# waveygang/wfmash

Measured on AMD Instinct MI355X. Metric: aligned bases/sec (whole node) + CIGAR-identical rate vs CPU ref, higher is better.
Workload: dtype int32; 1 GPU; C3: 64 synthetic 5%-divergence 50kb segment pairs per GPU, WFA-only (BiWFA gap-affine-2p 5,8,2,24,1; mappings pre-supplied); pairs_per_gpu=64, pairs_total=64, parallelism=records sharded over 1 GPU(s)

## Files before the change

### include/wfmash_hip.h

```cpp
#ifndef WFMASH_HIP_H_
#define WFMASH_HIP_H_

#include <stddef.h>
#include <stdint.h>

#ifdef __cplusplus
extern "C" {
#endif

#define WFM_OK              0
#define WFM_E_NODEVICE     (-1)
#define WFM_E_HIP          (-2)
#define WFM_E_ARG          (-3)
#define WFM_E_NOMEM        (-4)
#define WFM_E_UNSUPPORTED  (-5)
#define WFM_E_ARENA        (-6)

#define WFM_ST_OK            0
#define WFM_ST_UNREACHABLE (-300)
#define WFM_ST_OOM         (-200)
#define WFM_ST_MAX_SCORE   (-100)

#define WFMASH_HIP_VERSION "wfmash-hip-0.3"

// ... 164 lines not shown
#define WFM_COV_TILE 4096
#define WFM_COV_SCAN_BLOCK 1024
int  wfm_coverage_create(wfm_handle_t* h, uint64_t n_bases, wfm_coverage_t** cov);
void wfm_coverage_free(wfm_coverage_t* cov);
int  wfm_coverage_add(wfm_handle_t* h, wfm_coverage_t* cov, const wfm_cov_prob_t* probs, size_t n, const uint32_t* runs, size_t n_runs_total,
                      uint32_t* flags_out);
int  wfm_coverage_export(wfm_handle_t* h, wfm_coverage_t* cov, wfm_cov_entry_t** entries, size_t* n);
int  wfm_coverage_import(wfm_handle_t* h, wfm_coverage_t* cov, const wfm_cov_entry_t* entries, size_t n);
int  wfm_coverage_intervals(wfm_handle_t* h, wfm_coverage_t* cov, wfm_cov_interval_t** iv, size_t* n, uint64_t totals[3]);
void wfm_coverage_free_list(void* p);

typedef struct wfm_liftset wfm_liftset_t;
typedef struct { uint64_t start, end; } wfm_lift_iv_t;
typedef struct { uint32_t problem, interval, p0, p1, t0, t1, eq, x; } wfm_lift_t;
typedef struct { uint32_t flags, n_runs; uint64_t first, count; } wfm_liftcall_t;
#define WFM_LIFT_SPANS 2u
#define WFM_LIFT_SCAN_BLOCK 1024
int  wfm_liftset_create(wfm_handle_t* h, const wfm_lift_iv_t* iv, size_t n, uint64_t n_bases, wfm_liftset_t** out);
void wfm_liftset_free(wfm_liftset_t* s);
int  wfm_lift_runs(wfm_handle_t* h, const wfm_liftset_t* s, const wfm_cov_prob_t* probs, size_t n, const uint32_t* runs, size_t n_runs_total,
                   wfm_lift_t** lifts, size_t* n_lifts, wfm_liftcall_t* per);
void wfm_free_lifts(wfm_lift_t* p);

typedef struct wfm_pav wfm_pav_t;
typedef struct { uint64_t base, runs_off; uint32_t n_runs, group; } wfm_pav_prob_t;
typedef struct { uint64_t start; uint32_t length, group; } wfm_pav_seg_t;
#define WFM_PAV_SPANS 2u
#define WFM_PAV_SCAN_BLOCK 1024
int  wfm_pav_create(wfm_handle_t* h, uint64_t n_bases, uint32_t n_groups, wfm_pav_t** pav);
void wfm_pav_free(wfm_pav_t* pav);
int  wfm_pav_add(wfm_handle_t* h, wfm_pav_t* pav, const wfm_pav_prob_t* probs, size_t n, const uint32_t* runs, size_t n_runs_total,
                 uint32_t* flags_out);
int  wfm_pav_union(wfm_handle_t* h, wfm_pav_t* pav);
int  wfm_pav_export(wfm_handle_t* h, wfm_pav_t* pav, wfm_pav_seg_t** segs, size_t* n);
int  wfm_pav_import(wfm_handle_t* h, wfm_pav_t* pav, const wfm_pav_seg_t* segs, size_t n);
int  wfm_pav_matrix(wfm_handle_t* h, wfm_pav_t* pav, const wfm_lift_iv_t* iv, size_t n_iv, uint32_t* out);
int  wfm_pav_counts(const wfm_pav_t* pav, uint64_t out[3]);
void wfm_pav_free_list(void* p);

#define WFM_OPT_NOT_CHECKED 1u
#define WFM_OPT_SKIPPED     2u
#define WFM_OPT_CHEAPER     4u
#define WFM_OPT_UNREACHED   8u
typedef struct {
  uint32_t flags; int32_t dp_score;
  int32_t  band_lo, band_hi;
  uint64_t cells;
} wfm_optcheck_t;
#define WFM_OPT_BAND_C1   256
#define WFM_OPT_BAND_C4   1024
#define WFM_OPT_REG_MAX   4096
#define WFM_OPT_ROWS_MB   256
int wfm_check_optimal(wfm_handle_t* h, const wfm_penalties_t* pen, const wfm_seqset_t* s,
                      const wfm_result_t* res, uint64_t max_cells , wfm_optcheck_t* out);

void wfm_set_concurrent_calls(wfm_handle_t* h, int other_calls);

#define WFM_PF_ROOT_AGAIN   1u
#define WFM_PF_JOB_AGAIN    2u
#define WFM_PF_BASE_RETRY   4u
#define WFM_PF_BASE_RETRY2  8u
#define WFM_PF_BYTE_KERNEL 16u
#define WFM_PF_P2_ROUNDS   32u
#define WFM_PF_RING_KERNEL 64u
#define WFM_PF_BASE_TILES 128u
#define WFM_PF_RING_GROWN 256u
size_t wfm_get_problem_flags(const wfm_handle_t* h, uint32_t* out, size_t n);

enum {
  WFM_TC_JOBS = 0,
  WFM_TC_EXACT_ENDS = 1,
  WFM_TC_FINE_RERUNS = 2,
  WFM_TC_GAP_RERUNS = 3,
  WFM_TC_RING3 = 4,
  WFM_TC_BLOCKS_COARSE = 5,
  WFM_TC_BLOCKS_FINE = 6,
  WFM_TC_LEFT_BAND = 7,
  WFM_TC_REUSE_RESUMED = 8,
  WFM_TC_REUSE_FALLBACKS = 9,
  WFM_TC_REUSE_KEEPS = 10,
  WFM_TC_REUSE_TOUCHED = 11,
  WFM_TC_REUSE_FELL_OTHER = 12,
  WFM_TC_PLANNED_ENDS = 13,
  WFM_TILE_COUNTERS = 14
};
size_t wfm_get_tile_counters(const wfm_handle_t* h, uint64_t* out, size_t n);

size_t wfm_trim_device_cache(void);

int  wfm_get_stats(const wfm_handle_t* h, wfm_stats_t* out);
size_t wfm_get_busy_intervals(const wfm_handle_t* h, double* start_end_ms, size_t cap);


int  wfm_hash_kmers(wfm_handle_t* h, const char* seq, int64_t len, int k,
                    uint64_t* hash, int8_t* strand);

typedef struct {
  uint64_t hash;
  int64_t  wpos;
  int64_t  wpos_end;
  int32_t  seqId;
  int16_t  strand;
  int16_t  pad_;
} wfm_minmer_t;

int  wfm_sketch_fragments(wfm_handle_t* h, const char* seq, int64_t seq_len,
                          const int64_t* frag_off, const int32_t* frag_len, size_t n,
                          int k, int s, int32_t seq_id,
                          wfm_minmer_t* out, int32_t* out_count);

typedef struct {
  int64_t  pos;
  uint64_t hash;
  int32_t  seqId;
  int8_t   side;
  int8_t   pad_[3];
} wfm_interval_point_t;

typedef struct wfm_index wfm_index_t;
typedef struct {
  int64_t  n_windows;
  int64_t  n_kept;
  int64_t  n_unique;
  int64_t  n_points;
  uint64_t threshold;
  int64_t  filtered;
  int32_t  adjusted;
  int32_t  pad_;
} wfm_index_info_t;
int  wfm_index_build(wfm_handle_t* h, const wfm_minmer_t* minmers, int64_t n, double max_kmer_freq, wfm_index_t** out);
void wfm_index_free(wfm_handle_t* h, wfm_index_t* ix);
int  wfm_index_info(const wfm_index_t* ix, wfm_index_info_t* out);
int  wfm_index_download(wfm_handle_t* h, const wfm_index_t* ix, uint64_t* uhash, int64_t* poff,
                        wfm_interval_point_t* points, wfm_minmer_t* minmers);

int  wfm_index_replicate(wfm_handle_t* src, const wfm_index_t* ix, wfm_handle_t* dst, wfm_index_t** out);

int  wfm_index_upload(wfm_handle_t* h, const uint64_t* uhash, const int64_t* poff, int64_t n_unique,
                      const wfm_interval_point_t* points, const wfm_minmer_t* minmers, int64_t n_kept,
                      wfm_index_t** out);

int64_t wfm_add_minmers(wfm_handle_t* h, const char* seq, int64_t len, int k, int w, int s, int32_t seq_id,
                        wfm_minmer_t* out, int64_t cap);

int64_t wfm_add_minmers_multi(wfm_handle_t* h, const char* const* seqs, const int64_t* lens, const int32_t* seq_ids,
                              int64_t nseq, int k, int w, int s, int threads, wfm_minmer_t* out, int64_t cap, int64_t* counts);

int wfm_index_build_sequences(wfm_handle_t* h, const char* const* seqs, const int64_t* lens, const int32_t* seq_ids,
                              int64_t nseq, int k, int w, int s, int threads, double max_kmer_freq,
                              wfm_index_t** out, int64_t* n_windows);

typedef struct wfm_minmer_part wfm_minmer_part_t;
int  wfm_sketch_part(wfm_handle_t* h, const char* const* seqs, const int64_t* lens, const int32_t* seq_ids, int64_t nseq,
                     int k, int w, int s, int threads, wfm_minmer_part_t** out);
int64_t wfm_minmer_part_info(const wfm_minmer_part_t* part, int64_t* n_records, int64_t* counts, int64_t cap);
int64_t wfm_minmer_part_download(wfm_handle_t* h, const wfm_minmer_part_t* part, wfm_minmer_t* out, int64_t cap);
void wfm_minmer_part_free(wfm_minmer_part_t* part);

typedef struct { int32_t part; int32_t seq; } wfm_part_seq_t;
#define WFM_GATHER_TILE 2048
int  wfm_index_build_parts(wfm_handle_t* h, const wfm_minmer_part_t* const* parts, int nparts, const wfm_part_seq_t* order,
                           int64_t norder, double max_kmer_freq, wfm_index_t** out, int64_t* n_windows);

int64_t wfm_prefilter_kmers(wfm_handle_t* h, const char* seq, int64_t len, int k, int w, int s, double c_factor,
                            uint32_t* pos, uint64_t* hash, int8_t* strand, int64_t cap);

int64_t wfm_finish_records(wfm_handle_t* h, const wfm_minmer_t* raw, int64_t n, int w, wfm_minmer_t* out, int64_t cap,
// ... 90 lines not shown
```

### wfmash_amd/capi.py

```python
import ctypes as C
import os

import numpy as np

_HERE = os.path.dirname(os.path.abspath(__file__))
LIB_PATH = os.environ.get("WFM_LIB_PATH") or os.path.join(_HERE, "libwfmash_hip.so")

WFM_MODE_END2END_BIWFA = 0
WFM_MODE_ENDSFREE = 1
WFM_MODE_END2END_UNI = 2
WFM_MODE_MASK = 0xff
WFM_MODE_SCORE_ONLY = 0x100
WFM_MODE_SCORE_LIMIT = 0x200
WFM_ST_MAX_SCORE = -100

DEFAULT_PEN = (5, 8, 2, 24, 1)
WFM_PF_ROOT_AGAIN, WFM_PF_JOB_AGAIN, WFM_PF_BASE_RETRY, WFM_PF_BASE_RETRY2, WFM_PF_BYTE_KERNEL, WFM_PF_P2_ROUNDS, WFM_PF_RING_KERNEL, WFM_PF_BASE_TILES = 1, 2, 4, 8, 16, 32, 64, 128
WFM_PF_RING_GROWN = 256
TILE_COUNTERS = ("jobs", "exact_ends", "fine_reruns", "gap_reruns", "ring3", "blocks_coarse", "blocks_fine", "left_band",
                 "reuse_resumed", "reuse_fallbacks", "reuse_keeps", "reuse_touched", "reuse_fell_other", "planned_ends")

EXPORTS = [
    "wfm_create", "wfm_destroy", "wfm_last_error", "wfm_device_name",
    "wfm_align_arena_bytes", "wfm_align_batch", "wfm_upload_sequences",
    "wfm_free_sequences", "wfm_align_resident", "wfm_get_stats",
    "wfm_hash_kmers", "wfm_sketch_fragments", "wfm_add_minmers",
    "wfm_index_build", "wfm_index_free", "wfm_index_info", "wfm_index_download",
    "wfm_map_l1", "wfm_map_l2", "wfm_map_fragments", "wfm_minhash_sketch", "wfm_add_minmers_multi",
    "wfm_prefilter_kmers", "wfm_index_build_sequences", "wfm_index_upload",
    "wfm_index_replicate", "wfm_device_count", "wfm_finish_records",
    "wfm_align_batch_rle", "wfm_align_resident_rle", "wfm_free_runs", "wfm_score_bounds", "wfm_get_busy_intervals", "wfm_trim_device_cache", "wfm_map_fragments_ordered", "wfm_map_sequence_cache", "wfm_selftest_dpp", "wfm_selftest_arena_growth", "wfm_set_concurrent_calls", "wfm_get_problem_flags",
    "wfm_get_tile_counters",
    "wfm_streaming_minmers", "wfm_index_build_streaming",
    "wfm_sketch_part", "wfm_minmer_part_info", "wfm_minmer_part_download", "wfm_minmer_part_free", "wfm_index_build_parts",
    "wfm_seqstore_create", "wfm_seqstore_free", "wfm_seqstore_add", "wfm_seqstore_info",
    "wfm_upload_sequence_refs", "wfm_align_refs_rle", "wfm_download_sequences",
    "wfm_check_runs", "wfm_check_optimal", "wfm_left_align_runs", "wfm_cs_strings", "wfm_free_cs",
    "wfm_call_variants", "wfm_free_variants",
    "wfm_coverage_create", "wfm_coverage_free", "wfm_coverage_add", "wfm_coverage_export", "wfm_coverage_import", "wfm_coverage_intervals",
    "wfm_coverage_free_list",
    "wfm_liftset_create", "wfm_liftset_free", "wfm_lift_runs", "wfm_free_lifts",
    "wfm_pav_create", "wfm_pav_free", "wfm_pav_add", "wfm_pav_union", "wfm_pav_export", "wfm_pav_import", "wfm_pav_matrix", "wfm_pav_counts",
    "wfm_pav_free_list",
    "wfm_sketch_intersections",
]
ISECT_LDS_MAX = 4096
WFM_CK_NOT_CHECKED, WFM_CK_BAD_RUN, WFM_CK_SPANS, WFM_CK_M_DIFFERS, WFM_CK_X_EQUAL, WFM_CK_SCORE, WFM_CK_COUNTS = 1, 2, 4, 8, 16, 32, 64
CK_NAMES = ("NOT_CHECKED", "BAD_RUN", "SPANS", "M_DIFFERS", "X_EQUAL", "SCORE", "COUNTS")
CHECK_SLICE = 16384
WFM_LA_NOT_DONE, WFM_LA_SPANS = 1, 2
WFM_CS_SHORT, WFM_CS_LONG = 0, 1
WFM_CS_NOT_DONE, WFM_CS_SPANS = 1, 2
WFM_CS_SLICE = 16384
WFM_VAR_SNV, WFM_VAR_INS, WFM_VAR_DEL = 0, 1, 2
WFM_VAR_MASKED = 256
WFM_VAR_NOT_DONE, WFM_VAR_SPANS = 1, 2
WFM_VAR_SLICE = 16384
WFM_COV_SPANS = 2
WFM_COV_TILE = 4096
WFM_COV_SCAN_BLOCK = 1024
WFM_LIFT_SPANS = 2
WFM_LIFT_SCAN_BLOCK = 1024
WFM_PAV_SPANS = 2
WFM_PAV_SCAN_BLOCK = 1024
WFM_OPT_NOT_CHECKED, WFM_OPT_SKIPPED, WFM_OPT_CHEAPER, WFM_OPT_UNREACHED = 1, 2, 4, 8
OPT_NAMES = ("NOT_CHECKED", "SKIPPED", "CHEAPER", "UNREACHED")
OPT_BAND_C1, OPT_BAND_C4, OPT_REG_MAX = 256, 1024, 4096
OPT_ROWS_MB = 256
SEQ_GATHER_CHUNK = 16384


class Penalties(C.Structure):
    _fields_ = [("x", C.c_int32), ("o1", C.c_int32), ("e1", C.c_int32),
                ("o2", C.c_int32), ("e2", C.c_int32)]


class Problem(C.Structure):
    _fields_ = [("pattern", C.c_char_p), ("plen", C.c_int32),
                ("text", C.c_char_p), ("tlen", C.c_int32),
                ("mode", C.c_int32),
                ("pattern_begin_free", C.c_int32), ("pattern_end_free", C.c_int32),
                ("text_begin_free", C.c_int32), ("text_end_free", C.c_int32),
                ("score_hint", C.c_int32), ("pad_", C.c_int32)]


class ProblemRef(C.Structure):
    _fields_ = [("pattern", C.c_char_p), ("text", C.c_char_p),
                ("pattern_off", C.c_int64), ("text_off", C.c_int64),
                ("pattern_seq", C.c_int32), ("text_seq", C.c_int32),
                ("plen", C.c_int32), ("tlen", C.c_int32),
                ("mode", C.c_int32),
                ("pattern_revcomp", C.c_int32), ("text_revcomp", C.c_int32),
                ("pattern_begin_free", C.c_int32), ("pattern_end_free", C.c_int32),
                ("text_begin_free", C.c_int32), ("text_end_free", C.c_int32),
                ("score_hint", C.c_int32)]


class Result(C.Structure):
    _fields_ = [("status", C.c_int32), ("score", C.c_int32),
                ("ops_off", C.c_uint64), ("ops_len", C.c_uint32),
                ("n_runs", C.c_uint32), ("cells", C.c_uint64)]


# ... 2053 lines not shown
```

### wfmash_amd/csrc/wfa_device.h

```cpp
#ifndef WFM_WFA_DEVICE_H_
#define WFM_WFA_DEVICE_H_

#include <hip/hip_runtime.h>
#include <stdint.h>

#include "wfa_rows.h"

namespace wfm {

constexpr int WF_NULL = -(1 << 30);
constexpr int RING = 32;
constexpr int RMASK = RING - 1;
constexpr int RING_BIG = 128;

enum { C_M = 0, C_I1 = 1, C_I2 = 2, C_D1 = 3, C_D2 = 4 };
enum { OP_M = 0, OP_X = 1, OP_I = 2, OP_D = 3 };
enum { BT_I1_EXT = 8, BT_I2_EXT = 16, BT_D1_EXT = 32, BT_D2_EXT = 64 };

constexpr int WFM_DEV_UNREACHABLE = -300;
constexpr int WFM_DEV_OVERFLOW = -2;
constexpr int WFM_DEV_BAND = -4;
constexpr int WFM_DEV_P2_NOTHING = -6;
constexpr int WFM_DEV_LIMIT = -7;
constexpr int WFM_DEV_P2_MORE = -5;

struct DevPen { int x, o1, e1, o2, e2; };

struct BpJob {
  int64_t p_fwd, t_fwd, p_rev, t_rev;
  int64_t ring_off;
  int32_t pl, tl;
  int32_t comp_begin, comp_end;
  int32_t width;
  int32_t koff;
  int32_t resume_s;
  int32_t fmax0, rmax0;
  int32_t band;
  int32_t resume_sr;
  int32_t last_fwd;
  int32_t sub;
  int32_t best0;
  int32_t packed;
  int32_t limit;
};
static_assert(sizeof(BpJob) == 104, "BpJob::limit fills the struct's tail padding: the job arrays keep their stride");

struct TileJob {
  int64_t p_fwd, t_fwd, p_rev, t_rev;
  int64_t ring_in, ring_out;
  int32_t pl, tl;
  int32_t comp_begin, comp_end;
  int32_t width, koff;
  int32_t s0;
  int32_t active;
  int32_t fmax, rmax;
  int32_t nblocks;
  int32_t mode;
  int32_t tf, tr;
  int32_t last_fwd;
  int32_t packed;
  int64_t p2_off;
  int32_t w2, koff2;
  int32_t sub;
  int32_t fine_s;
  int64_t ring_prev;
  int32_t prev_ok;
  int32_t reran;
  int32_t plan_sum;
  int32_t plan_deep;
};
static_assert(sizeof(TileJob) == 160, "TileJob::plan_sum and its padding behind reran: no field the tile kernels read has moved");
__host__ __device__ inline bool tile_plan_enter(TileJob& J, int T) {
  if (J.plan_sum <= 0) return false;
  const int sf = (J.plan_sum + 1) / 2, sr = J.plan_sum / 2;
  if ((sf - 1) / T * T != J.s0) return false;
  J.tf = sf - J.s0; J.tr = sr - J.s0; J.last_fwd = J.plan_sum & 1;
  J.mode = (J.ring_prev >= 0 && J.prev_ok && !J.plan_deep && (J.tf < J.tr ? J.tf : J.tr) < 26) ? 6 : 1;
  return true;
}
__host__ __device__ inline bool tile_plan_short_next(const TileJob& J, int T) {
  if (J.plan_sum <= 0 || !J.plan_deep || J.mode != 0) return false;
  const int sf = (J.plan_sum + 1) / 2, sr = J.plan_sum / 2, b0 = (sf - 1) / T * T;
  return b0 == J.s0 + T && sr - b0 < 26;
}

struct KeepTask {
  int32_t* dst;
  int32_t job, dir;
  int32_t expect_s;
  int32_t kmin, n;
  int32_t pad_;
};
struct RestoreTask {
  const int32_t* src;
  int32_t job, dir;
  int32_t s_k, kmin, n;
  int32_t slack;
};
void launch_keep(const int32_t* ring, const TileJob* jobs, const KeepTask* tasks, int ntasks, int max_n, hipStream_t st);
void launch_restore(int32_t* ring, const TileJob* jobs, const RestoreTask* tasks, int32_t* out, int ntasks, int max_n, hipStream_t st);

constexpr int P2K = 32;
constexpr int P2ROWS = SNAP_ROWS + P2K;
constexpr int P2TESTS = 2 * P2K;
constexpr int P2ENT = RING * 5;
struct P2Job {
  int64_t ring_in;
  int64_t p2_off;
  int32_t width, koff;
  int32_t w2, koff2;
  int32_t pl, tl;
  int32_t sf, sr, last_fwd;
  int32_t sub, best0;
  int32_t nblk;
  int64_t bm_off;
};

struct BpResult {
  int32_t status;
  int32_t score, score_fwd, score_rev, k_fwd, off_fwd, comp;
  int32_t steps;
  uint64_t cells;
  int32_t steps_p1;
  uint32_t ticks_p1, ticks_p2;
  int32_t pad_;
  uint32_t ticks_list, ticks_pick;
  uint32_t work_items, pad2_;
};

struct BaseJob {
  int64_t p_off, t_off;
  int64_t pre_off;
  int64_t bt_off;
  int64_t ring_off;
  int64_t rle_end;
  int32_t pl, tl;
  int32_t comp_begin, comp_end;
  int32_t endsfree, pbf, pef, tbf, tef;
  int32_t smax, kmin, width;
  int32_t type;
  int32_t pad_;
  int32_t score_only;
};
static_assert(sizeof(BaseJob) == 112, "BaseJob::score_only fills the struct's tail padding: the job arrays keep their stride");

struct BaseResult {
  int32_t status;
  int32_t score;
  int32_t nruns;
  int32_t pad_;
  uint64_t cells;
};

struct Base2TJob {
  BaseJob b;
  int64_t snap_in, snap_out;
  int32_t ntiles, core;
  int32_t task0;
  int32_t s0;
  int32_t done;
  int32_t end_s, end_k, end_off;
};
struct Base2TTask { int32_t job, tile; };
constexpr int B2T_ROWS = 32;
constexpr int B2T_THREADS = 512;
void launch_base2t_block(const uint32_t* pk, int32_t* a32, uint8_t* a8, const Base2TJob* jobs, const Base2TTask* tasks, unsigned long long* tile_key,
                         int32_t* tile_off, int ntasks, int T, hipStream_t st);
void launch_base2t_advance(Base2TJob* jobs, const unsigned long long* tile_key, const int32_t* tile_off, int njobs, int T, int32_t* active_slot, hipStream_t st);
void launch_base2t_finish(const int32_t* a32, const uint8_t* a8, uint32_t* rle, const Base2TJob* jobs, BaseResult* res, int njobs, hipStream_t st);

struct BoundJob { int64_t p_off, t_off; int32_t pl, tl; };
void launch_bound(const uint8_t* seq, const BoundJob* jobs, int32_t* out, int njobs, DevPen pen, hipStream_t st);

struct SeqRev { int64_t p_fwd, p_rev, t_fwd, t_rev; int32_t plen, tlen; };
void launch_reverse(uint8_t* seq, const SeqRev* jobs, int njobs, int pad, hipStream_t st);
struct SeqGatherTask { const uint8_t* src; uint8_t* dst; int32_t len, pad; int32_t reverse, complement; };
void launch_seq_gather(const SeqGatherTask* tasks, int64_t ntasks, hipStream_t st);
struct CheckProb {
  int64_t p_off, t_off;
  uint64_t run_off;
  uint32_t n_runs;
  int32_t plen, tlen;
  int32_t pbf, pef, tbf, tef;
  int32_t res_score;
  uint32_t res_ops_len;
  int32_t skip;
};
struct CheckTask { int32_t prob, slice; };
void launch_check(const uint8_t* seq, const uint32_t* runs, const CheckProb* probs, int nprob, const CheckTask* tasks, int64_t ntasks,
                  uint32_t* ops_pre, uint32_t* p_pre, uint32_t* t_pre, uint32_t* cmp_ops, unsigned long long* keys, void* out, DevPen pen,
                  hipStream_t st);
struct LaProb {
  int64_t p_off, t_off;
  uint64_t run_off, out_off, gap_off;
  uint32_t n_runs, n_gaps;
  int32_t plen, tlen;
  int32_t skip, pad_;
};
struct LaGap { int64_t s_off; uint32_t g, len, prob, run; };
// ... 18 lines not shown
                      hipStream_t st);
struct CovProb {
  uint64_t base, runs_off;
  uint32_t n_runs, pad_;
};
void launch_cov_add(const uint32_t* runs, const CovProb* probs, int nprob, int32_t* d, unsigned long long n_bases, uint32_t* flags, hipStream_t st);
void launch_cov_tile_offsets(const int32_t* d, unsigned long long ntiles, uint32_t* tile_cnt, unsigned long long* sums, unsigned long long* tile_off,
                             hipStream_t st);
void launch_cov_write(const int32_t* d, const unsigned long long* tile_off, unsigned long long tile_a, unsigned long long tile_b,
                      unsigned long long out_base, void* out, hipStream_t st);
void launch_cov_import(const void* ent, unsigned long long n, int32_t* d, hipStream_t st);
void launch_cov_intervals(const void* ent, unsigned long long m, unsigned long long* sums, unsigned long long* carry, unsigned long long prev_pos,
                          unsigned long long n_bases, int last, void* iv, unsigned long long* totals, hipStream_t st);
struct LiftProb {
  uint64_t base, runs_off, pre_off;
  uint32_t n_runs, pad_;
};
struct LiftWin {
  uint64_t lo, hi, count;
  uint32_t flags, plen;
};
void launch_lift_pm(const void* iv, unsigned long long n, unsigned long long* maxs, unsigned long long* pm, hipStream_t st);
void launch_lift_index(const uint32_t* runs, const LiftProb* probs, int nprob, const void* iv, const unsigned long long* pm, unsigned long long n_iv,
                       unsigned long long n_bases, void* pre, LiftWin* win, unsigned long long* off, hipStream_t st);
void launch_lift_write(const uint32_t* runs, const LiftProb* probs, const void* iv, const void* pre, const LiftWin* win, const unsigned long long* off,
                       uint32_t ka, uint32_t kb, void* out, hipStream_t st);
struct PavProb {
  uint64_t base, runs_off;
  uint32_t n_runs, group;
};
void launch_pav_count(const uint32_t* runs, const PavProb* probs, int nprob, unsigned long long n_bases, uint32_t n_groups, uint32_t* flags,
                      unsigned long long* cnt, unsigned long long* off, hipStream_t st);
void launch_pav_write(const uint32_t* runs, const PavProb* probs, int nprob, const uint32_t* flags, const unsigned long long* off,
                      unsigned long long* ks, unsigned long long* ke, hipStream_t st);
hipError_t pav_sort(void* tmp, size_t* tmp_bytes, const unsigned long long* ks, unsigned long long* ks2, const unsigned long long* ke,
                    unsigned long long* ke2, unsigned long long n, unsigned end_bit, hipStream_t st);
void launch_pav_runmax(unsigned long long* ke, unsigned long long n, unsigned long long* aux, hipStream_t st);
void launch_pav_compact(const unsigned long long* ks, const unsigned long long* rm, unsigned long long n, unsigned long long* aux,
                        unsigned long long* uks, unsigned long long* uke, hipStream_t st);
void launch_pav_prefix(const unsigned long long* uks, const unsigned long long* uke, unsigned long long m, unsigned long long* aux,
                       unsigned long long* C, hipStream_t st);
void launch_pav_matrix(const unsigned long long* uks, const unsigned long long* uke, const unsigned long long* C, unsigned long long m, const void* iv,
                       unsigned long long ra, unsigned long long rb, uint32_t n_groups, uint32_t* out, hipStream_t st);
struct OptProb {
  int64_t p_off, t_off, row_off;
  int32_t plen, tlen;
  int32_t pbf, pef, tbf, tef;
  int32_t band_lo, band_hi;
};
void launch_optcheck(const uint8_t* seq, const OptProb* probs, int nprob, int form, int32_t* rows, int32_t* out, DevPen pen, hipStream_t st);
void launch_seq_normalize(uint8_t* seq, int64_t nbytes, hipStream_t st);
void launch_seq_pack(const uint8_t* seq, uint32_t* pk, int64_t nwords, int64_t nbytes, const SeqRev* jobs, int njobs, int32_t* flag, hipStream_t st);
constexpr int64_t PK_PAD_WORDS = 2048 + 64;
void launch_tile2(const uint32_t* pk, int32_t* ring, const TileJob* jobs, const TileTask* tasks, int32_t* mak, int ntasks, int threads, int T, int variants, hipStream_t st);
#ifndef WFM_TILE_SLOTS_WIDE
#define WFM_TILE_SLOTS_WIDE 16
#endif
constexpr int TILE_SLOTS_WAVE1 = 2, TILE_SLOTS_SMALL = 4, TILE_SLOTS_WIDE = WFM_TILE_SLOTS_WIDE;
constexpr int tile_fine_slots(int threads) { return threads <= 64 ? TILE_SLOTS_WAVE1 : (threads <= 128 ? TILE_SLOTS_SMALL : TILE_SLOTS_WIDE); }
bool tile2_coarse_maxima();
void launch_tile2_p2(const uint32_t* pk, int32_t* ring, const TileJob* jobs, const TileTask* tasks, int ntasks, int threads, int32_t* p2, hipStream_t st);
int selftest_dpp(int* host_out128, hipStream_t st);
void launch_base2(const uint32_t* pk, int32_t* a32, uint8_t* a8, uint32_t* rle, const BaseJob* jobs, BaseResult* res, int njobs, int threads, hipStream_t st);
void launch_bp(const uint8_t* seq, int32_t* ring, const BpJob* jobs, BpResult* res, int njobs, int threads,
               DevPen pen, int scope, int ring_rows, hipStream_t st);
void launch_tile_init(const uint8_t* seq, int32_t* ring, const TileJob* jobs, int32_t* mak0, int njobs, int ring_rows, hipStream_t st);
void launch_tile(const uint8_t* seq, int32_t* ring, const TileJob* jobs, const TileTask* tasks, int32_t* mak, int ntasks,
                 int threads, int T, int Wt, size_t lds_bytes, DevPen pen, int scope, int ring_rows, hipStream_t st);
void launch_tile_advance(TileJob* jobs, int32_t* mak, int njobs, int T, DevPen pen, int exact, int coarse, int launched, hipStream_t st);
void launch_tile_reg(const uint8_t* seq, int32_t* ring, const TileJob* jobs, const TileTask* tasks, int32_t* mak, int ntasks,
                     int threads, int T, int C, bool cut, hipStream_t st);
void launch_tile_p2(const uint8_t* seq, int32_t* ring, const TileJob* jobs, const TileTask* tasks, int ntasks, int threads,
                    int32_t* p2, bool cut, hipStream_t st);
void launch_p2_to_ring(int32_t* ring, const int32_t* p2, const P2Job* jobs, int njobs, hipStream_t st);
struct RingWidenJob {
  const int32_t* src;
  int32_t* dst;
  int32_t src_w, src_koff;
  int32_t dst_w, dst_koff;
  int32_t klo, khi;
};
void launch_ring_widen(const RingWidenJob* jobs, int njobs, int max_dst_w, int ring_rows, hipStream_t st);
void launch_p2_blockmax(const int32_t* ring, const int32_t* p2, const P2Job* jobs, int32_t* bmax, int32_t* p2max, int njobs, hipStream_t st);
void launch_p2_overlap(const int32_t* ring, const int32_t* p2, const P2Job* jobs, const int32_t* p2max, const int32_t* bmax, int32_t* pbmax,
                       BpResult* res, int njobs, int threads, int max_nblk, DevPen pen, int scope, hipStream_t st);
void launch_base(const uint8_t* seq, int32_t* a32, uint8_t* a8, uint32_t* rle, const BaseJob* jobs, BaseResult* res,
                 int njobs, DevPen pen, bool wide, int ring_rows, hipStream_t st);
void launch_compact(const uint32_t* rle, const int64_t* off, const int64_t* cap, uint32_t* out, unsigned long long* total,
                    int64_t* out_start, int32_t* out_count, int nprob, hipStream_t st);

}
#endif
```

### wfmash_amd/csrc/wfa_host.hip

```cpp
#include <hip/hip_runtime.h>

#include <algorithm>
#include <chrono>
#include <climits>
#include <cstdio>
#include <cstring>
#include <atomic>
#include <mutex>
#include <string>
#include <thread>
#include <vector>

#include "../../include/wfmash_hip.h"
#include "wfa_host_shared.h"
#include "wfa_plan.h"
#include "wfa_optband.h"

#ifdef WFM_PROFILE_SECTIONS
namespace wfm { void read_sections(long long* out); }
#endif
namespace wfm { void p2_counters(unsigned long long* out); }
namespace {

using namespace wfm;
// ... 774 lines not shown
  wfm_handle* h = p.h;
  uint64_t unique_level = 0;
  for (size_t i = 0; i < p.n; ++i) {
    const TileJob& t = p.tj[i];
    const int sf_end = t.mode == 2 ? t.s0 + t.tf : t.s0, sr_end = t.mode == 2 ? t.s0 + t.tr : t.s0;
    if (p.ru && p.ru->bad[i]) continue;
    unique_level += (uint64_t)cells_sum(t.pl, t.tl, t.sub, p.s_begin[i] + 1, sf_end) + (uint64_t)cells_sum(t.pl, t.tl, t.sub, p.s_begin[i] + 1, sr_end);
  }
  h->stats.cells_tile_unique += unique_level;
  for (size_t i = 0; i < p.n; ++i) {
    const TileJob& t = p.tj[i];
    BpJob& j = p.jobs[(size_t)p.tiled[i]];
    j.ring_off = t.ring_in;
    p.ring2[i] = t.ring_out;
    j.resume_s = t.s0;
    j.resume_sr = -1; j.last_fwd = 0;
    h->tile_ctr[WFM_TC_EXACT_ENDS] += t.mode == 2;
    h->tile_ctr[WFM_TC_PLANNED_ENDS] += t.mode == 2 && t.plan_sum > 0;
    h->tile_ctr[WFM_TC_LEFT_BAND] += t.mode == 3 && !(p.ru && p.ru->bad[i]);
    if (t.mode == 3) {
      j.resume_s = -3; j.resume_sr = t.s0; j.fmax0 = p.fmax[i]; j.rmax0 = p.rmax[i];
      continue;
    }
    if (t.mode == 2) {
      j.resume_s = t.s0 + t.tf;
      j.resume_sr = t.s0 + t.tr;
      j.last_fwd = t.last_fwd;
    }
    j.fmax0 = p.fmax[i]; j.rmax0 = p.rmax[i];
  }
  if (p.cfg.debug) fprintf(stderr, "[wfm] level %u: tiled %zu jobs, %u blocks of %d scores (Wt %d), %.3f ms; %.3e cells computed on %.3e lane-steps (%.0f %% of the lanes hold a cell), %.3e of them in the result (the block in which a job's wavefronts meet runs twice); launches of the packed kernel without / with per-score maxima %u / %u, mode-5 reruns %u, mode-6 reruns %u\n", level, p.n, p.blocks, p.T, p.cfg.Wt, p.tile_ms,
                           (double)p.tile_cells - cells_before, p.lane_cells, p.lane_cells > 0 ? 100.0 * ((double)p.tile_cells - cells_before) / p.lane_cells : 0.0, (double)unique_level,
                           p.launches_coarse, p.launches_fine, p.reruns5, p.reruns6);
}

int run_tiled_phase(wfm_handle* h, wfm_seqset* S, const DevPen& dp, int scope, const TileCfg& cfg, int T, bool refine,
                    std::vector<BpJob>& jobs, const std::vector<int>& tiled, std::vector<int64_t>& ring2,
                    double& tile_ms, uint64_t& tile_cells, uint32_t level, const std::vector<int32_t>* fine_from = nullptr,
                    const std::vector<int64_t>* ring3 = nullptr, ReuseCtl* reuse = nullptr, const std::vector<int32_t>* plan_from = nullptr) {
  const size_t n = tiled.size();
  if (n == 0) return WFM_OK;
  const double cells_before = (double)tile_cells;
  TilePhase p{h, S, dp, scope, cfg, T, refine, jobs, tiled, ring2, tile_ms, tile_cells, n};
  p.ru = refine ? nullptr : reuse;
  int rc = init_tile_jobs(p, fine_from, ring3, plan_from);
  if (rc != WFM_OK) return rc;
  if (p.n_active) {
    HIPCHK(h, hipMemcpyAsync(h->tilejobs.p, p.tj.data(), n * sizeof(TileJob), hipMemcpyHostToDevice, h->stream));
    HIPCHK(h, hipMemsetAsync(h->tilemak.p, 0, n * 2 * (size_t)T * sizeof(int32_t), h->stream));
    p.chunk = std::max(1, std::min(cfg.chunk, (int)h->tile_ev.size() / 2));
    p.got.resize(n); p.pjobs.resize(n);
    p.rules = TilePlanRules{cfg.threads, cfg.C, T, p.chunk, cfg.Wt - 2 * T, cfg.reg, cfg.fine, cfg.reg && cfg.exact && tile2_coarse_maxima(), p.any_planned};
    auto clk = [] { return std::chrono::steady_clock::now(); };
    auto msd = [](std::chrono::steady_clock::time_point a, std::chrono::steady_clock::time_point b) { return std::chrono::duration<double, std::milli>(b - a).count(); };
    double ms_prep = 0, ms_launch = 0, ms_wait = 0, ms_post = 0;
    while (p.n_active) {
      const auto tq0 = clk();
      if ((rc = drop_leavers(p)) != WFM_OK) return rc;
      if (!p.n_active) break;
      if ((rc = plan_tile_tasks(p)) != WFM_OK) return rc;
      const auto tq1 = clk();
      if ((rc = launch_chunk(p)) != WFM_OK) return rc;
      const auto tq2 = clk();
      HIPCHK(h, hipStreamSynchronize(h->stream));
      const auto tq3 = clk();
      if ((rc = time_chunk(p)) != WFM_OK) return rc;
      account_chunk(p);
      settle_keeps(p);
      if ((rc = restore_kept(p)) != WFM_OK) return rc;
      ms_prep += msd(tq0, tq1); ms_launch += msd(tq1, tq2); ms_wait += msd(tq2, tq3); ms_post += msd(tq3, clk());
    }
    if (cfg.debug > 1)
      fprintf(stderr, "[wfm] level %u tile phase, host side: task lists %.2f ms, launches %.2f ms, waiting for the device %.2f ms, bookkeeping %.2f ms\n", level, ms_prep, ms_launch, ms_wait, ms_post);
  }
  hand_back(p, level, cells_before);
  return WFM_OK;
}


struct P2Chunk {
  wfm_handle* h; wfm_seqset* S; const DevPen& dp; int scope; const TileCfg& cfg; std::vector<BpJob>& jobs;
  const std::vector<int>& cand; const std::vector<int64_t>& ring_other; std::vector<BpResult>& res; double& ms_out;
  std::vector<BpResult>& carry; std::vector<char>& has_carry; bool may_continue; std::vector<int>& again;
  std::vector<P2PlanJob> pcand;
  P2ChunkPlan plan;
  size_t i0 = 0, n = 0;
  std::vector<TileJob> tj;
  std::vector<P2Job> pj;
  std::vector<BpResult> got;
  float ms = 0;
};

void fill_p2_chunk(P2Chunk& c, size_t i0) {
  const size_t budget = std::max<size_t>(c.h->mem_budget / 4, (size_t)64 << 20);
  plan_p2_chunk(c.pcand.data(), c.pcand.size(), i0, P2K, P2ROWS, budget, c.cfg.threads, c.cfg.Wt - 2 * P2K, c.plan);
  c.i0 = i0; c.n = c.plan.geo.size();
  c.tj.clear(); c.pj.clear();
  for (size_t q = 0; q < c.n; ++q) {
    const BpJob& j = c.jobs[(size_t)c.cand[i0 + q]];
    const P2Geometry& g = c.plan.geo[q];
    TileJob t = tile_job_from(j);
    t.ring_out = c.ring_other[i0 + q];
    t.mode = 4; t.tf = j.resume_s; t.tr = j.resume_sr; t.last_fwd = j.last_fwd;
    t.p2_off = (int64_t)g.p2_off; t.w2 = (int32_t)g.w2; t.koff2 = g.koff2;
    P2Job pq{};
    pq.ring_in = j.ring_off; pq.p2_off = (int64_t)g.p2_off; pq.width = j.width; pq.koff = j.koff; pq.w2 = (int32_t)g.w2; pq.koff2 = g.koff2;
    pq.pl = j.pl; pq.tl = j.tl; pq.sf = j.resume_s; pq.sr = j.resume_sr; pq.last_fwd = j.last_fwd; pq.sub = j.sub; pq.best0 = j.best0;
    pq.nblk = (int32_t)g.nblk; pq.bm_off = (int64_t)g.bm_off;
    c.tj.push_back(t); c.pj.push_back(pq);
  }
}

int launch_p2_chunk(P2Chunk& c) {
  wfm_handle* h = c.h;
  wfm_seqset* S = c.S;
  const size_t n = c.n, elems = c.plan.elems, bm_elems = c.plan.bm_elems, n_pk = c.plan.tiles.n_pk;
  const std::vector<TileTask>& tasks = c.plan.tiles.tasks;
  const int threads_c = c.plan.threads_c;
  if (h->p2rows.ensure(elems + 16) || h->p2max.ensure(n * 2 * P2ROWS * 5) || h->p2bmax.ensure(bm_elems + 16) || h->p2pbmax.ensure(bm_elems + 16) ||
      h->p2jobs.ensure(n) || h->tilejobs.ensure(n) || h->tiletasks.ensure(tasks.size()) || h->bpres.ensure(std::max(n, c.jobs.size()))) {
    h->err = "out of device memory (phase-2 rows)"; return WFM_E_NOMEM;
  }
  HIPCHK(h, hipMemcpyAsync(h->tilejobs.p, c.tj.data(), n * sizeof(TileJob), hipMemcpyHostToDevice, h->stream));
  HIPCHK(h, hipMemcpyAsync(h->p2jobs.p, c.pj.data(), n * sizeof(P2Job), hipMemcpyHostToDevice, h->stream));
  HIPCHK(h, hipMemcpyAsync(h->tiletasks.p, tasks.data(), tasks.size() * sizeof(TileTask), hipMemcpyHostToDevice, h->stream));
  HIPCHK(h, hipEventRecord(h->ev0, h->stream));
  bool any_cut = false;
  for (const TileJob& t : c.tj) any_cut |= t.sub != SUB_NONE;
  if (n_pk) launch_tile2_p2(S->d_pk, h->ring.p, h->tilejobs.p, h->tiletasks.p, (int)n_pk, threads_c, h->p2rows.p, h->stream);
  if (tasks.size() > n_pk) launch_tile_p2(S->d_seq, h->ring.p, h->tilejobs.p, h->tiletasks.p + n_pk, (int)(tasks.size() - n_pk), threads_c, h->p2rows.p, any_cut, h->stream);
  launch_p2_blockmax(h->ring.p, h->p2rows.p, h->p2jobs.p, h->p2bmax.p, h->p2max.p, (int)n, h->stream);
  static const int p2_threads = getenv("WFM_P2_THREADS") ? atoi(getenv("WFM_P2_THREADS")) : 0;
  launch_p2_overlap(h->ring.p, h->p2rows.p, h->p2jobs.p, h->p2max.p, h->p2bmax.p, h->p2pbmax.p, h->bpres.p, (int)n,
                    p2_threads > 0 ? p2_threads : 1024, (int)(c.plan.maxw2 >> 6) + 1, c.dp, c.scope, h->stream);
  HIPCHK(h, hipGetLastError());
  HIPCHK(h, hipEventRecord(h->ev1, h->stream));
  c.got.resize(n);
  HIPCHK(h, hipMemcpyAsync(c.got.data(), h->bpres.p, n * sizeof(BpResult), hipMemcpyDeviceToHost, h->stream));
  HIPCHK(h, hipStreamSynchronize(h->stream));
  HIPCHK(h, hipEventElapsedTime(&c.ms, h->ev0, h->ev1));
  c.ms_out += c.ms;
  if (h->call_base) {
    float t0 = 0;
    HIPCHK(h, hipEventElapsedTime(&t0, h->call_base, h->ev0));
    h->bp_iv.emplace_back(t0, t0 + c.ms);
  }
  return WFM_OK;
}

int dump_p2_job(P2Chunk& c) {
  wfm_handle* h = c.h;
  const std::vector<BpResult>& got = c.got;
  const size_t q = std::min<size_t>((size_t)c.cfg.p2_dump, c.n - 1);
  std::vector<int32_t> rm((size_t)2 * P2ROWS * 5);
  HIPCHK(h, hipMemcpy(rm.data(), h->p2max.p + q * 2 * P2ROWS * 5, rm.size() * 4, hipMemcpyDeviceToHost));
  const P2Job& pjq = c.pj[q];
  fprintf(stderr, "[wfm] p2 dump job %zu: pl %d tl %d sf %d sr %d last_fwd %d sub %d w2 %d nblk %d -> status %d score %d (fwd %d rev %d comp %d k %d) rounds %d\n", q, pjq.pl, pjq.tl, pjq.sf,
          pjq.sr, pjq.last_fwd, pjq.sub, pjq.w2, pjq.nblk, got[q].status, got[q].score, got[q].score_fwd, got[q].score_rev, got[q].comp, got[q].k_fwd, got[q].pad_);
  for (int d = 0; d < 2; ++d)
    for (int r = 0; r < P2ROWS; r += 3) {
      const int32_t* m = rm.data() + ((size_t)d * P2ROWS + r) * 5;
      fprintf(stderr, "[wfm]   dir %d row %d (s = %d): max M %d I1 %d I2 %d D1 %d D2 %d\n", d, r, (d == 0 ? pjq.sf : pjq.sr) - RNG_BACK + r, m[0], m[1], m[2], m[3], m[4]);
    }
  return WFM_OK;
}

void print_p2_chunk(const P2Chunk& c) {
  const std::vector<BpResult>& got = c.got;
  const std::vector<P2Job>& pj = c.pj;
  const size_t n = c.n;
  int more = 0;
  double tk = 0, tc = 0, rd = 0; uint32_t tkmax = 0; int rdmax = 0;
  for (const BpResult& r : got) { more += r.status == WFM_DEV_P2_MORE; tk += r.ticks_p2; tc += r.ticks_p1; rd += r.pad_; tkmax = std::max(tkmax, r.ticks_p2); rdmax = std::max(rdmax, r.pad_); }
  fprintf(stderr, "[wfm] phase 2 from rows computed ahead: %zu jobs, widest %zu columns, %zu tiles of %d threads, %.3f ms, %d left to the step kernel; walk per job: %.1f rounds (max %d), %.0f us (max %.0f), of which cells stage %.0f us\n",
          n, c.plan.maxw2, c.plan.tiles.tasks.size(), c.plan.threads_c, c.ms, more, rd / n, rdmax, tk / n / 100.0, tkmax / 100.0, tc / n / 100.0);
  size_t qs = 0;
  for (size_t q = 0; q < n; ++q) if (got[q].ticks_p2 > got[qs].ticks_p2) qs = q;
  fprintf(stderr, "[wfm]   slowest walk: pl %d tl %d sub %d w2 %d nblk %d: %d rounds, %.0f us = listing %.0f + cells %.0f (incl. listing) + pick %.0f, %u blocks listed, status %d\n", pj[qs].pl, pj[qs].tl,
          pj[qs].sub == SUB_NONE ? -1 : pj[qs].sub, pj[qs].w2, pj[qs].nblk, got[qs].pad_, got[qs].ticks_p2 / 100.0, got[qs].ticks_list / 100.0, got[qs].ticks_p1 / 100.0, got[qs].ticks_pick / 100.0,
          got[qs].work_items, got[qs].status);
}

int continue_p2_chunk(P2Chunk& c) {
  wfm_handle* h = c.h;
  std::vector<BpResult>& got = c.got;
  std::vector<P2Job> mj;
  for (size_t q = 0; q < c.n; ++q) {
    const size_t jq = (size_t)c.cand[c.i0 + q];
    BpJob& j = c.jobs[jq];
    if (got[q].status == WFM_DEV_P2_NOTHING) { got[q] = c.carry[jq]; continue; }
    if (got[q].status != WFM_DEV_P2_MORE) continue;
    if (got[q].comp >= 0) {
      c.carry[jq] = got[q]; c.carry[jq].status = 0; c.has_carry[jq] = 1;
      j.best0 = got[q].score;
    }
    if (!c.may_continue || (j.band > 0 && std::max(j.resume_s, j.resume_sr) + 2 * P2K + 2 > j.band)) continue;
    mj.push_back(c.pj[q]);
    j.resume_s += P2K; j.resume_sr += P2K;
    c.again.push_back((int)(c.i0 + q));
  }
  if (!mj.empty()) {
    HIPCHK(h, hipMemcpyAsync(h->p2jobs.p, mj.data(), mj.size() * sizeof(P2Job), hipMemcpyHostToDevice, h->stream));
    launch_p2_to_ring(h->ring.p, h->p2rows.p, h->p2jobs.p, (int)mj.size(), h->stream);
    HIPCHK(h, hipGetLastError());
    HIPCHK(h, hipStreamSynchronize(h->stream));
  }
  for (size_t q = 0; q < c.n; ++q) c.res[(size_t)c.cand[c.i0 + q]] = got[q];
  return WFM_OK;
}

int run_p2_phase(wfm_handle* h, wfm_seqset* S, const DevPen& dp, int scope, const TileCfg& cfg, std::vector<BpJob>& jobs,
                 const std::vector<int>& cand, const std::vector<int64_t>& ring_other, std::vector<BpResult>& res, double& ms_out,
                 std::vector<BpResult>& carry, std::vector<char>& has_carry, bool may_continue, std::vector<int>& again) {
  if (cand.empty()) return WFM_OK;
  P2Chunk c{h, S, dp, scope, cfg, jobs, cand, ring_other, res, ms_out, carry, has_carry, may_continue, again};
  for (int q : cand) {
    const BpJob& j = jobs[(size_t)q];
    c.pcand.push_back(P2PlanJob{j.pl, j.tl, j.sub, j.resume_s, j.resume_sr, j.packed});
  }
  for (size_t i0 = 0; i0 < cand.size(); i0 += c.n) {
    fill_p2_chunk(c, i0);
    int rc = launch_p2_chunk(c);
    if (rc != WFM_OK) return rc;
    if (cfg.p2_dump_on && (rc = dump_p2_job(c)) != WFM_OK) return rc;
    h->stats.p2_launches++;
    h->stats.p2_jobs += (uint32_t)c.n;
    if (cfg.debug) print_p2_chunk(c);
    if ((rc = continue_p2_chunk(c)) != WFM_OK) return rc;
  }
  return WFM_OK;
}


struct Knobs {
  static int num(const char* name, int dflt) { const char* e = getenv(name); return e ? atoi(e) : dflt; }
  bool use_hints = num("WFM_SCORE_HINT", 1) != 0;
  bool use_bound = use_hints && num("WFM_BOUND", 1) != 0;
  int slack_env = num("WFM_SUB_SLACK", -1);
  bool ring3_on = num("WFM_TILE_RING3", 1) != 0, p2_on = num("WFM_P2", 1) != 0;
  int p2_rounds = std::max(1, num("WFM_P2_ROUNDS", 64));
  int fine_margin = num("WFM_TILE_FINE_MARGIN", 48);
  int coarse_min_blocks = num("WFM_TILE_COARSE_MIN_BLOCKS", 32), coarse_max_jobs = num("WFM_TILE_COARSE_MAX_JOBS", 128);
  bool planned_end = num("WFM_TILE_PLANNED_END", 1) != 0 && slack_env < (1 << 28);
  bool tile_v2 = num("WFM_TILE_V2", 1) != 0;
  bool band_on = num("WFM_BAND", 1) != 0;
  int band_root = std::max(64, num("WFM_BAND_ROOT", 4096));
  int resume_margin = num("WFM_RESUME_MARGIN", SNAP_ROWS);
  bool reuse = num("WFM_REUSE", 1) != 0 && slack_env < (1 << 28);
  int reuse_min_blocks = std::max(1, num("WFM_REUSE_MIN_BLOCKS", 8));
  int reuse_every = std::max(1, num("WFM_REUSE_EVERY", 2)), reuse_slack = std::max(0, num("WFM_REUSE_TOUCH_SLACK", 0));
  int reuse_levels = num("WFM_REUSE_LEVELS", 8);
  int debug = env_debug();
};

struct Chunk {
  std::vector<BpJob> jobs;
  std::vector<int32_t> node_of;
  size_t ring_elems = 0, end = 0;
  int maxw = 0;
  std::vector<int> tiled, tiled_r;
  std::vector<int64_t> ring2, ring3, ring2_r;
  std::vector<int32_t> fine_from, fine_r, snap_r;
  std::vector<int32_t> plan_from;
  std::vector<size_t> ring_third;
  std::vector<char> grown_job, resume_bad, has_carry;
  std::vector<ReuseUse> reuse;
  std::vector<int32_t> keep_upto;
  std::vector<char> reuse_bad;
  std::vector<std::vector<int32_t>> kept[2];
  std::vector<BpResult> res, carry;
  std::vector<int> rest, more_set;
  void clear() {
    jobs.clear(); node_of.clear(); ring_elems = 0; maxw = 0;
    tiled.clear(); ring2.clear(); ring3.clear(); ring_third.clear(); fine_from.clear();
    tiled_r.clear(); ring2_r.clear(); fine_r.clear(); snap_r.clear(); grown_job.clear();
    reuse.clear(); keep_upto.clear(); plan_from.clear();
  }
};

struct AlignCall {
  wfm_handle* h;
  const wfm_penalties_t* pen;
  wfm_seqset* S;
  size_t first, last;
  wfm_result_t* out;
  char* ops_arena;
  size_t arena_bytes, arena_base;
  std::vector<uint32_t>* runs_out;
  uint32_t* pflags;
  int scope;
  DevPen dp;
  const Knobs knobs;
  TileCfg tcfg;
  BaseCfg bcfg;
  int RR;
  RingRules rules;
  std::vector<int32_t> prob_status;
  std::vector<uint64_t> prob_cells;
  std::vector<int32_t> prob_score;
  std::vector<Node> bp_nodes, base_nodes, next_bp;
  uint32_t level = 0;
  Chunk ck;
  LevelTimer tm;
  double wall_tile = 0, wall_base = 0;
  uint64_t band_retries = 0, band_jobs = 0, roots_banded = 0, roots_out = 0, hint_retries = 0, limit_out = 0;
  uint64_t grown_jobs = 0, grown_widened = 0, grown_restarts = 0;
  int64_t grown_maxband = 0;
  size_t ring_peak = 0;
  GrownSnaps snaps;
  KeepStore keeps;
  uint64_t reuse_children = 0, reuse_found = 0, reuse_taken = 0;
  uint64_t keep_bytes = 0, restore_bytes = 0;
  uint64_t reuse_full_rings = 0;
};

void make_roots(AlignCall& c) {
  for (size_t i = c.first; i < c.last; ++i) {
    const ProbMeta& pm = c.S->meta[i];
    Node nd{};
    nd.prob = (int32_t)i; nd.pb = 0; nd.pl = pm.plen; nd.tb = 0; nd.tl = pm.tlen;
    nd.cb = C_M; nd.ce = C_M; nd.score_rem = INT_MAX; nd.endsfree = 0;
    nd.sub = SUB_NONE; nd.hinted = 0;
// ... 175 lines not shown
  k.resume_bad.assign(k.jobs.size(), 0);
  if (k.tiled_r.empty()) return WFM_OK;
  std::vector<RingWidenJob> wj;
  int maxw_dst = 0;
  for (size_t q = 0; q < k.tiled_r.size(); ++q) {
    BpJob& j = k.jobs[(size_t)k.tiled_r[q]];
    const GrownSnap& sn = c.snaps.v[(size_t)k.snap_r[q] - 1];
    wj.push_back(RingWidenJob{sn.d, h->ring.p + j.ring_off, sn.w, sn.koff, j.width, j.koff, -(sn.s0 + 8), sn.s0 + 8});
    maxw_dst = std::max(maxw_dst, j.width);
    j.resume_s = sn.s0; j.resume_sr = -1; j.fmax0 = sn.fmax; j.rmax0 = sn.rmax;
  }
  if (h->widenjobs.ensure(wj.size())) { h->err = "out of device memory (ring arena)"; return WFM_E_NOMEM; }
  HIPCHK(h, hipMemcpyAsync(h->widenjobs.p, wj.data(), wj.size() * sizeof(RingWidenJob), hipMemcpyHostToDevice, h->stream));
  launch_ring_widen(h->widenjobs.p, (int)wj.size(), maxw_dst, c.RR, h->stream);
  HIPCHK(h, hipGetLastError());
  HIPCHK(h, hipStreamSynchronize(h->stream));
  for (int32_t id : k.snap_r) c.snaps.drop(id);
  return WFM_OK;
}

int run_chunk_tiles(AlignCall& c) {
  wfm_handle* h = c.h;
  Chunk& k = c.ck;
  const TileCfg& tcfg = c.tcfg;
  double tms = 0; uint64_t tcells = 0;
  const auto tw0 = std::chrono::steady_clock::now();
  ReuseCtl ru;
  ru.store = &c.keeps; ru.slack = c.knobs.reuse_slack; ru.min_blocks = c.knobs.reuse_min_blocks;
  ru.use = k.reuse; ru.upto = k.keep_upto;
  for (size_t q = 0; q < k.tiled.size(); ++q) {
    const Node& nd = c.bp_nodes[(size_t)k.node_of[(size_t)k.tiled[q]]];
    ru.meet.push_back(nd.score_rem != INT_MAX ? nd.score_rem / 2 : 0);
  }
  {
    std::vector<ReuseKeeper> kp;
    for (size_t q = 0; q < k.tiled.size(); ++q) {
      const BpJob& j = k.jobs[(size_t)k.tiled[q]];
      if (k.keep_upto[q] > 0) kp.push_back(ReuseKeeper{j.pl, j.tl, k.keep_upto[q] == INT_MAX ? (j.pl + j.tl) / 16 : k.keep_upto[q]});
    }
    c.keeps.cap_bytes = h->mem_budget / 8;
    const int chunk_blocks = std::max(1, std::min(tcfg.chunk, (int)h->tile_ev.size() / 2));
    ru.cadence = kp.empty() ? 0 : reuse_fit_cadence(kp.data(), kp.size(), reuse_cadence(c.knobs.reuse_every, chunk_blocks), tcfg.T, c.keeps.cap_bytes);
  }
  const bool any_reuse = ru.cadence > 0 || std::any_of(ru.use.begin(), ru.use.end(), [](const ReuseUse& u) { return u.keep > 0; });
  int rc = run_tiled_phase(h, c.S, c.dp, c.scope, tcfg, tcfg.T, false, k.jobs, k.tiled, k.ring2, tms, tcells, c.level, &k.fine_from, &k.ring3, any_reuse ? &ru : nullptr, &k.plan_from);
  k.reuse_bad.assign(k.jobs.size(), 0);
  k.kept[0].assign(k.jobs.size(), {}); k.kept[1].assign(k.jobs.size(), {});
  if (any_reuse && !ru.bad.empty())
    for (size_t q = 0; q < k.tiled.size(); ++q) {
      k.reuse_bad[(size_t)k.tiled[q]] = ru.bad[q];
      for (int d = 0; d < 2; ++d) k.kept[d][(size_t)k.tiled[q]].swap(ru.kept[d][q]);
    }
  c.keep_bytes += ru.keep_bytes; c.restore_bytes += ru.restore_bytes;
  if (rc == WFM_OK && tcfg.T_refine > 0 && tcfg.T_refine < tcfg.T && !(tcfg.reg && tcfg.exact))
    rc = run_tiled_phase(h, c.S, c.dp, c.scope, tcfg, tcfg.T_refine, true, k.jobs, k.tiled, k.ring2, tms, tcells, c.level);
  if (rc == WFM_OK && !k.tiled_r.empty()) {
    std::vector<int> from_s(k.tiled_r.size());
    for (size_t q = 0; q < k.tiled_r.size(); ++q) from_s[q] = k.jobs[(size_t)k.tiled_r[q]].resume_s;
    rc = run_tiled_phase(h, c.S, c.dp, c.scope, tcfg, tcfg.T, true, k.jobs, k.tiled_r, k.ring2_r, tms, tcells, c.level, &k.fine_r);
    for (size_t q = 0; rc == WFM_OK && q < k.tiled_r.size(); ++q) {
      BpJob& j = k.jobs[(size_t)k.tiled_r[q]];
      const bool exact_end = j.resume_s >= 0 && j.resume_sr >= 0;
      if (tcfg.reg && tcfg.exact && ((exact_end && std::min(j.resume_s, j.resume_sr) - from_s[q] < c.knobs.resume_margin) || (j.resume_s >= 0 && j.resume_sr < 0 && j.resume_s == from_s[q]))) {
        j.resume_s = -3; j.resume_sr = -1;
        k.resume_bad[(size_t)k.tiled_r[q]] = 1;
      }
      k.tiled.push_back(k.tiled_r[q]); k.ring2.push_back(k.ring2_r[q]);
    }
  }
  c.wall_tile += std::chrono::duration<double, std::milli>(std::chrono::steady_clock::now() - tw0).count();
  if (rc != WFM_OK) return rc;
  c.tm.bp_ms += tms; c.tm.tile_ms += tms;
  h->stats.cells_bp += tcells; h->stats.cells_tile += tcells;
  return WFM_OK;
}

int run_chunk_p2(AlignCall& c) {
  wfm_handle* h = c.h;
  Chunk& k = c.ck;
  k.res.assign(k.jobs.size(), BpResult{});
  k.rest.clear(); k.more_set.clear();
  std::vector<int> cand;
  std::vector<int64_t> other;
  std::vector<char> is_cand(k.jobs.size(), 0);
  if (c.knobs.p2_on && c.tcfg.reg && c.tcfg.exact)
    for (size_t q = 0; q < k.tiled.size(); ++q) {
      const BpJob& j = k.jobs[(size_t)k.tiled[q]];
      if (j.resume_s >= 0 && j.resume_sr >= 0) { cand.push_back(k.tiled[q]); other.push_back(k.ring2[q]); is_cand[(size_t)k.tiled[q]] = 1; }
    }
  double pms = 0;
  k.carry.assign(k.jobs.size(), BpResult{});
  k.has_carry.assign(k.jobs.size(), 0);
  std::vector<int> cand_r = cand, again;
  std::vector<int64_t> other_r = other;
  for (int round = 1; !cand_r.empty(); ++round) {
    again.clear();
    const int rc = run_p2_phase(h, c.S, c.dp, c.scope, c.tcfg, k.jobs, cand_r, other_r, k.res, pms, k.carry, k.has_carry, round < c.knobs.p2_rounds, again);
    if (rc != WFM_OK) return rc;
    std::vector<int> c2; std::vector<int64_t> o2;
    for (int a : again) {
      c2.push_back(cand_r[(size_t)a]); o2.push_back(other_r[(size_t)a]);
      if (c.pflags) c.pflags[c.bp_nodes[(size_t)k.node_of[(size_t)cand_r[(size_t)a]]].prob] |= WFM_PF_P2_ROUNDS;
    }
    h->stats.p2_again += (uint32_t)again.size();
    cand_r.swap(c2); other_r.swap(o2);
  }
  c.tm.bp_ms += pms;
  for (size_t q = 0; q < k.jobs.size(); ++q)
    if (!is_cand[q] || k.res[q].status == WFM_DEV_P2_MORE) { k.rest.push_back((int)q); h->stats.p2_more += is_cand[q]; if (is_cand[q]) k.more_set.push_back((int)q); }
  if (c.pflags)
    for (size_t q = 0; q < k.jobs.size(); ++q)
      if (is_cand[q] && k.res[q].status == WFM_DEV_P2_MORE) c.pflags[c.bp_nodes[(size_t)k.node_of[q]].prob] |= WFM_PF_P2_ROUNDS;
  return WFM_OK;
}

int run_chunk_step(AlignCall& c) {
  wfm_handle* h = c.h;
  Chunk& k = c.ck;
  const std::vector<int>& rest = k.rest;
  if (rest.empty()) return WFM_OK;
  auto is_more = [&](int q) { return std::find(k.more_set.begin(), k.more_set.end(), q) != k.more_set.end(); };
  int threads = 1024;
  if (k.maxw <= 1024) threads = 256;
  else if (k.maxw <= 8192) threads = 512;
  std::vector<BpJob> rj(rest.size());
  for (size_t q = 0; q < rest.size(); ++q) rj[q] = k.jobs[(size_t)rest[q]];
  HIPCHK(h, hipMemcpyAsync(h->bpjobs.p, rj.data(), rj.size() * sizeof(BpJob), hipMemcpyHostToDevice, h->stream));
  HIPCHK(h, hipEventRecord(h->ev0, h->stream));
  launch_bp(c.S->d_seq, h->ring.p, h->bpjobs.p, h->bpres.p, (int)rj.size(), threads, c.dp, c.scope, c.RR, h->stream);
  HIPCHK(h, hipGetLastError());
  HIPCHK(h, hipEventRecord(h->ev1, h->stream));
  std::vector<BpResult> rr(rj.size());
  HIPCHK(h, hipMemcpyAsync(rr.data(), h->bpres.p, rr.size() * sizeof(BpResult), hipMemcpyDeviceToHost, h->stream));
  HIPCHK(h, hipStreamSynchronize(h->stream));
  float ms = 0;
  HIPCHK(h, hipEventElapsedTime(&ms, h->ev0, h->ev1));
  c.tm.bp_ms += ms;
  if (h->call_base) {
    float t0 = 0;
    HIPCHK(h, hipEventElapsedTime(&t0, h->call_base, h->ev0));
    h->bp_iv.emplace_back(t0, t0 + ms);
  }
  h->stats.bp_launches++;
  for (size_t q = 0; q < rest.size(); ++q) {
    if (rr[q].status == WFM_DEV_P2_NOTHING) {
      const uint64_t cl = rr[q].cells; const int32_t st = rr[q].steps;
      rr[q] = k.carry[(size_t)rest[q]]; rr[q].cells = cl; rr[q].steps = st;
    }
    k.res[(size_t)rest[q]] = rr[q];
  }
  if (c.knobs.debug) {
    uint64_t cl = 0; double t1 = 0, t2 = 0; int64_t st1 = 0, st = 0; uint32_t m1 = 0, m2 = 0;
    for (const BpResult& r : rr) { cl += r.cells; t1 += r.ticks_p1; t2 += r.ticks_p2; st1 += r.steps_p1; st += r.steps; m1 = std::max(m1, r.ticks_p1); m2 = std::max(m2, r.ticks_p2); }
    fprintf(stderr, "[wfm] level %u: %zu bp jobs (step kernel), %d thr, %.3f ms, cells %.3e, avg steps p1 %.0f p2 %.0f, avg ms p1 %.3f p2 %.3f, max ms p1 %.3f p2 %.3f\n", c.level, rr.size(), threads, ms,
            (double)cl, (double)st1 / rr.size(), (double)(st - st1) / rr.size(), t1 / rr.size() / 1e5, t2 / rr.size() / 1e5, m1 / 1e5, m2 / 1e5);
    if (c.knobs.debug > 1) {
      std::vector<size_t> ord(rr.size());
      for (size_t q = 0; q < ord.size(); ++q) ord[q] = q;
      std::sort(ord.begin(), ord.end(), [&](size_t a, size_t b) { return rr[a].ticks_p1 + rr[a].ticks_p2 > rr[b].ticks_p1 + rr[b].ticks_p2; });
      for (size_t q = 0; q < std::min<size_t>(3, ord.size()); ++q) {
        const BpResult& r = rr[ord[q]];
        const BpJob& j = rj[ord[q]];
        fprintf(stderr, "[wfm]   slow step-kernel job: pl %d tl %d width %d band %d sub %d resume %d/%d (%s), status %d score %d = %d + %d, steps p1 %d p2 %d, ms p1 %.3f p2 %.3f\n", j.pl, j.tl, j.width,
                j.band, j.sub == SUB_NONE ? -1 : j.sub, j.resume_s, j.resume_sr, is_more(rest[ord[q]]) ? "phase-2 walk ran out of rows" : (j.resume_sr >= 0 ? "exact" : "not exact"), r.status,
                r.score, r.score_fwd, r.score_rev, r.steps_p1, r.steps - r.steps_p1, r.ticks_p1 / 1e5, r.ticks_p2 / 1e5);
      }
    }
  }
  return WFM_OK;
}

int keep_snapshot(AlignCall& c, size_t q, Node& again) {
  wfm_handle* h = c.h;
  const BpJob& j = c.ck.jobs[q];
  if (c.ck.resume_bad[q] || c.ck.res[q].status != WFM_DEV_BAND || j.resume_s != -3 || j.resume_sr < 0 || j.sub != SUB_NONE || j.band <= 0) return WFM_OK;
  GrownSnap sn;
  sn.s0 = j.resume_sr; sn.fmax = j.fmax0; sn.rmax = j.rmax0;
  const int reach = sn.s0 + 8;
  sn.koff = reach + 4;
  sn.koff += ((j.koff - sn.koff) % 4 + 4) % 4;
// ... 282 lines not shown
  GatheredRuns g;
  bool any_full = false;
  for (size_t i = first; i < last && !any_full; ++i) any_full = !S->meta[i].score_only();
  if (any_full && (rc = gather_runs(c, g)) != WFM_OK) return rc;
  uint64_t cells_total = 0;
  const int failed = write_results(c, g, &cells_total);
  if (failed < 0) return failed;
  cells_total += h->stats.cells_tile;
  h->stats.cells = cells_total;
  uint64_t range_bases = 0;
  for (size_t i = first; i < last; ++i) range_bases += (uint64_t)S->meta[i].plen + (uint64_t)S->meta[i].tlen;
  h->stats.bytes_algorithmic = 48ull * cells_total + range_bases;
  h->stats.ms_breakpoint = c.tm.bp_ms;
  h->stats.ms_tile = c.tm.tile_ms;
  h->stats.ms_base = c.tm.base_ms;
  h->stats.ms_kernels = c.tm.bp_ms + c.tm.base_ms;
  h->stats.ms_total = std::chrono::duration<double, std::milli>(std::chrono::steady_clock::now() - t_start).count();
  if (c.knobs.debug)
    fprintf(stderr, "[wfm] wall: total %.2f ms | levels %.2f (tile phase %.2f incl. kernels %.2f; base phase %.2f incl. kernels %.2f; bp kernels %.2f) | gather+expand %.2f\n",
            h->stats.ms_total, std::chrono::duration<double, std::milli>(t_levels - t_start).count(), c.wall_tile, c.tm.tile_ms, c.wall_base, c.tm.base_ms,
            c.tm.bp_ms - c.tm.tile_ms, std::chrono::duration<double, std::milli>(std::chrono::steady_clock::now() - t_levels).count());
  return failed;
}

}

extern "C" {

int wfm_device_count(void) {
  int ndev = 0;
  if (hipGetDeviceCount(&ndev) != hipSuccess) { (void)hipGetLastError(); return 0; }
  return ndev < 0 ? 0 : ndev;
}

int wfm_create(int device, wfm_handle_t** out) {
  if (!out) return WFM_E_ARG;
  *out = nullptr;
  int ndev = 0;
  if (hipGetDeviceCount(&ndev) != hipSuccess || ndev <= 0) return WFM_E_NODEVICE;
  if (device < 0 || device >= ndev) return WFM_E_ARG;
  if (hipSetDevice(device) != hipSuccess) return WFM_E_HIP;
  hipDeviceProp_t prop;
  if (hipGetDeviceProperties(&prop, device) != hipSuccess) return WFM_E_HIP;
  if (strncmp(prop.gcnArchName, "gfx9", 4) != 0 || prop.warpSize != 64) return WFM_E_NODEVICE;
  wfm_handle* h = new wfm_handle();
  h->device = device;
  h->name = prop.name[0] ? std::string(prop.name) + " (" + prop.gcnArchName + ")" : std::string(prop.gcnArchName);
  if (hipStreamCreate(&h->stream) != hipSuccess) { delete h; return WFM_E_HIP; }
  (void)hipEventCreate(&h->ev0); (void)hipEventCreate(&h->ev1); (void)hipEventCreate(&h->ev2); (void)hipEventCreate(&h->ev3);
  h->tile_ev.resize(64);
  for (auto& e : h->tile_ev) (void)hipEventCreate(&e);
  (void)hipEventCreate(&h->ev_base);
  size_t fr = 0, tot = 0;
  if (hipMemGetInfo(&fr, &tot) != hipSuccess) { fr = (size_t)16 << 30; }
  wfm_dcache_warm();
  int live = 0;
  { std::lock_guard<std::mutex> lk(g_base_mu); if (device < 64) live = g_dev_handles[device]++; }
  h->mem_budget = std::min<size_t>((size_t)((double)fr * 0.40 / (double)(1 + live)), (size_t)32 << 30);
  const char* env = getenv("WFM_MEM_BUDGET_MB");
  if (env) h->mem_budget = (size_t)atoll(env) << 20;
  h->mem_budget_full = h->mem_budget;
  *out = h;
  return WFM_OK;
}

void wfm_destroy(wfm_handle_t* h) {
  if (!h) return;
  for (wfm_handle* p : h->peers) wfm_destroy(p);
  h->peers.clear();
  bool last_of_process = false;
  if (!h->is_peer) {
    std::lock_guard<std::mutex> lk(g_base_mu);
    if (h->device < 64 && g_dev_handles[h->device] > 0) --g_dev_handles[h->device];
    last_of_process = true;
    for (int d = 0; d < 64; ++d) last_of_process &= g_dev_handles[d] == 0;
  }
  (void)hipSetDevice(h->device);
  h->ring.release(); h->base32.release(); h->base8.release(); h->rle.release(); h->rle_out.release();
  h->tilejobs.release(); h->tiletasks.release(); h->tilemak.release();
  h->revjobs.release(); h->bndjobs.release(); h->bndres.release();
  if (h->stage) { (void)hipHostFree(h->stage); h->stage = nullptr; h->stage_cap = 0; }
  for (int k = 0; k < 2; ++k)
    if (h->cspin[k]) { (void)hipHostFree(h->cspin[k]); h->cspin[k] = nullptr; }
  h->p2rows.release(); h->p2max.release(); h->p2bmax.release(); h->p2pbmax.release(); h->p2jobs.release(); h->widenjobs.release(); h->keeptasks.release(); h->restoretasks.release(); h->restoreres.release();
  h->bpjobs.release(); h->bpres.release(); h->bsjobs.release(); h->bsres.release();
  h->b2tjobs.release(); h->b2ttasks.release(); h->b2tkeys.release(); h->b2toffs.release(); h->b2tactive.release();
  h->i64a.release(); h->i64b.release(); h->i64c.release(); h->i32a.release(); h->seqflags.release(); h->flagjobs.release(); h->gathertasks.release(); h->scratch.release(); h->outblk.release(); h->optrows.release(); h->total.release();
  if (h->ev0) (void)hipEventDestroy(h->ev0);
  if (h->ev1) (void)hipEventDestroy(h->ev1);
  if (h->ev2) (void)hipEventDestroy(h->ev2);
  if (h->ev3) (void)hipEventDestroy(h->ev3);
  for (auto& e : h->tile_ev) if (e) (void)hipEventDestroy(e);
  if (h->ev_base) (void)hipEventDestroy(h->ev_base);
  if (h->attachment && h->attachment_free) h->attachment_free(h->attachment);
  if (h->stream) (void)hipStreamDestroy(h->stream);
  delete h;
  if (last_of_process && g_last_handle_hook) {
    std::lock_guard<std::mutex> lk(g_base_mu);
    bool still_last = true;
    for (int d = 0; d < 64; ++d) still_last &= g_dev_handles[d] == 0;
    if (still_last) g_last_handle_hook();
  }
}

const char* wfm_last_error(const wfm_handle_t* h) { return h ? h->err.c_str() : "null handle"; }

void wfm_set_concurrent_calls(wfm_handle_t* h, int other_calls) { if (h) h->other_calls = other_calls > 0 ? other_calls : 0; }

size_t wfm_get_problem_flags(const wfm_handle_t* h, uint32_t* out, size_t n) {
  if (!h) return 0;
  const size_t have = h->prob_flags.empty() ? 0 : h->prob_flags.size() - 1;
  if (out) for (size_t i = 0; i < n && i < have; ++i) out[i] = h->prob_flags[i];
  return have;
}

size_t wfm_get_tile_counters(const wfm_handle_t* h, uint64_t* out, size_t n) {
  if (!h) return 0;
  if (out) for (size_t i = 0; i < n && i < (size_t)WFM_TILE_COUNTERS; ++i) out[i] = h->tile_ctr[i];
  return (size_t)WFM_TILE_COUNTERS;
}

int wfm_device_name(const wfm_handle_t* h, char* buf, size_t buflen) {
  if (!h || !buf || !buflen) return WFM_E_ARG;
  snprintf(buf, buflen, "%s", h->name.c_str());
  return WFM_OK;
}

size_t wfm_align_arena_bytes(const wfm_problem_t* problems, size_t n) {
  size_t t = 0;
  for (size_t i = 0; i < n; ++i)
    if (!(problems[i].mode & WFM_MODE_SCORE_ONLY)) t += (size_t)problems[i].plen + (size_t)problems[i].tlen + 1;
  return t;
}

}
namespace {
template <typename P>
int check_modes(wfm_handle* h, const P* problems, size_t n) {
  for (size_t i = 0; i < n; ++i) {
    const int32_t mode = problems[i].mode, m = mode & WFM_MODE_MASK;
    const char* what = nullptr;
    if (mode & ~(WFM_MODE_MASK | WFM_MODE_SCORE_ONLY | WFM_MODE_SCORE_LIMIT)) what = "unknown bits in mode";
    else if (m != WFM_MODE_END2END_BIWFA && m != WFM_MODE_ENDSFREE && m != WFM_MODE_END2END_UNI) what = "unknown mode";
    else if ((mode & WFM_MODE_SCORE_LIMIT) && m != WFM_MODE_END2END_BIWFA) what = "WFM_MODE_SCORE_LIMIT takes END2END_BIWFA";
    else if ((mode & WFM_MODE_SCORE_LIMIT) && problems[i].score_hint <= 0) what = "WFM_MODE_SCORE_LIMIT takes a score_hint > 0";
    if (what) { h->err = "problem " + std::to_string(i) + ": " + what; return WFM_E_ARG; }
  }
  return WFM_OK;
}

template <typename P>
void layout_seqset(wfm_seqset* S, const P* problems, size_t n, size_t* fwd_bytes_out) {
  S->meta.resize(n);
  size_t bytes = SEQ_PAD, rev_bytes = 0;
  int64_t rle = 0;
  for (size_t i = 0; i < n; ++i) {
    const P& p = problems[i];
    ProbMeta& m = S->meta[i];
    m.plen = p.plen; m.tlen = p.tlen; m.mode = p.mode & WFM_MODE_MASK; m.flags = p.mode & ~WFM_MODE_MASK;
    m.limit = (m.flags & WFM_MODE_SCORE_LIMIT) ? p.score_hint : 0;
    m.hint = (m.mode == WFM_MODE_END2END_BIWFA && p.score_hint > 0 && !m.limit) ? p.score_hint : 0;
    m.pbf = std::min(std::max(p.pattern_begin_free, 0), p.plen); m.pef = std::min(std::max(p.pattern_end_free, 0), p.plen);
    m.tbf = std::min(std::max(p.text_begin_free, 0), p.tlen);    m.tef = std::min(std::max(p.text_end_free, 0), p.tlen);
    if (m.mode != WFM_MODE_ENDSFREE) { m.pbf = m.pef = m.tbf = m.tef = 0; }
    m.p_fwd = (int64_t)bytes; bytes += (size_t)p.plen + SEQ_PAD;
    m.t_fwd = (int64_t)bytes; bytes += (size_t)p.tlen + SEQ_PAD;
    const bool need_rev = (m.mode == WFM_MODE_END2END_BIWFA);
// ... 648 lines not shown
```

### wfmash_amd/csrc/wfa_host_shared.h

```cpp
#ifndef WFM_WFA_HOST_SHARED_H_
#define WFM_WFA_HOST_SHARED_H_
#include <hip/hip_runtime.h>

#include <algorithm>
#include <chrono>
#include <cstdio>
#include <cstdlib>
#include <string>
#include <vector>

#include "../../include/wfmash_hip.h"
#include "wfa_device.h"
#include "dev_cache.h"

#define HIPCHK(h, call)                                                                 \
  do {                                                                                  \
    hipError_t e_ = (call);                                                             \
    if (e_ != hipSuccess) {                                                             \
      (h)->err = std::string(#call) + ": " + hipGetErrorString(e_);                     \
      return WFM_E_HIP;                                                                 \
    }                                                                                   \
  } while (0)

namespace wfm {
// ... 6 lines not shown
    if (n <= cap) return 0;
    const size_t old_cap = cap;
    if (p) wfm_dfree(p);
    p = nullptr; cap = 0;
    size_t want = std::max(n + n / 8 + 64, std::min(old_cap * 2, n + ((size_t)8 << 30) / sizeof(T)));
    const auto t0 = std::chrono::steady_clock::now();
    if (wfm_dmalloc((void**)&p, want * sizeof(T)) != hipSuccess) {
      (void)hipGetLastError();
      if (wfm_dmalloc((void**)&p, n * sizeof(T)) != hipSuccess) { (void)hipGetLastError(); p = nullptr; return -1; }
      want = n;
    }
    cap = want;
    if (want * sizeof(T) >= ((size_t)256 << 20) && getenv("WFM_DEBUG"))
      fprintf(stderr, "[wfm] device block of %.2f GB took %.1f ms\n", (double)(want * sizeof(T)) / 1073741824.0,
              std::chrono::duration<double, std::milli>(std::chrono::steady_clock::now() - t0).count());
    return 0;
  }
  void release() { if (p) wfm_dfree(p); p = nullptr; cap = 0; }
};

struct ProbMeta {
  int64_t p_fwd, t_fwd, p_rev, t_rev;
  int32_t plen, tlen;
  int32_t mode, pbf, pef, tbf, tef;
  int32_t hint;
  int64_t rle_off;
  int32_t flags;
  int32_t limit;
  bool score_only() const { return (flags & WFM_MODE_SCORE_ONLY) != 0; }
};

inline int env_num(const char* name, int dflt) { const char* e = getenv(name); return e ? atoi(e) : dflt; }
inline int env_debug() { return getenv("WFM_DEBUG") ? std::max(1, env_num("WFM_DEBUG", 0)) : 0; }

inline int validate_pen(const wfm_penalties_t* pen, int* scope) {
  if (!pen) return WFM_E_ARG;
  if (pen->x <= 0 || pen->e1 <= 0 || pen->e2 <= 0 || pen->o1 < 0 || pen->o2 < 0) return WFM_E_UNSUPPORTED;
  const int sc = std::max(pen->x, std::max(pen->o1 + pen->e1, pen->o2 + pen->e2)) + 1;
  if (sc > RING_BIG - 2) return WFM_E_UNSUPPORTED;
  *scope = sc;
  return WFM_OK;
}

}

struct wfm_seqset {
  uint8_t* d_seq = nullptr;
  uint32_t* d_pk = nullptr;
  std::vector<int32_t> acgt;
  size_t bytes = 0;
  std::vector<wfm::ProbMeta> meta;
  int64_t rle_total = 0;
  uint64_t seq_bases = 0;
};

struct wfm_handle {
  int device = 0;
  std::vector<std::pair<double, double>> busy_abs;
  hipStream_t stream = nullptr;
  hipEvent_t ev0 = nullptr, ev1 = nullptr, ev2 = nullptr, ev3 = nullptr;
  std::vector<hipEvent_t> tile_ev;
  std::vector<wfm_handle*> peers;
  bool is_peer = false;
  hipEvent_t ev_base = nullptr;
  hipEvent_t call_base = nullptr;
  std::vector<std::pair<float, float>> tile_iv;
  std::vector<std::pair<float, float>> bp_iv, base_iv;
  std::string err;
  std::string name;
  std::vector<uint32_t> prob_flags;
  int other_calls = 0;
  size_t mem_budget = 0;
  size_t mem_budget_full = 0;
  wfm_stats_t stats{};
  uint64_t tile_ctr[WFM_TILE_COUNTERS] = {};
  wfm::DevBuf<int32_t> ring;
  wfm::DevBuf<int32_t> base32;
  wfm::DevBuf<uint8_t> base8;
  wfm::DevBuf<uint32_t> rle, rle_out;
  wfm::DevBuf<wfm::BpJob> bpjobs;
  wfm::DevBuf<wfm::TileJob> tilejobs;
  wfm::DevBuf<wfm::TileTask> tiletasks;
  wfm::DevBuf<int32_t> tilemak;
  wfm::DevBuf<int32_t> p2rows, p2max, p2bmax, p2pbmax;
  wfm::DevBuf<wfm::P2Job> p2jobs;
  wfm::DevBuf<wfm::RingWidenJob> widenjobs;
  wfm::DevBuf<wfm::KeepTask> keeptasks;
  wfm::DevBuf<wfm::RestoreTask> restoretasks;
  wfm::DevBuf<int32_t> restoreres;
  wfm::DevBuf<wfm::SeqRev> revjobs;
  wfm::DevBuf<wfm::BoundJob> bndjobs;
  wfm::DevBuf<int32_t> bndres;
  uint8_t* stage = nullptr;
  size_t stage_cap = 0;
  wfm::DevBuf<wfm::BpResult> bpres;
  wfm::DevBuf<wfm::BaseJob> bsjobs;
  wfm::DevBuf<wfm::BaseResult> bsres;
  wfm::DevBuf<wfm::Base2TJob> b2tjobs;
  wfm::DevBuf<wfm::Base2TTask> b2ttasks;
  wfm::DevBuf<unsigned long long> b2tkeys;
  wfm::DevBuf<int32_t> b2toffs, b2tactive;
  wfm::DevBuf<int64_t> i64a, i64b, i64c;
  wfm::DevBuf<int32_t> i32a;
  wfm::DevBuf<int32_t> seqflags;
  wfm::DevBuf<wfm::SeqRev> flagjobs;
  wfm::DevBuf<wfm::SeqGatherTask> gathertasks;
  uint8_t* cspin[2] = {nullptr, nullptr};
  wfm::DevBuf<uint64_t> scratch;
  wfm::DevBuf<uint64_t> outblk;
  wfm::DevBuf<int32_t> optrows;
  wfm::DevBuf<unsigned long long> total;
  void* attachment = nullptr;
  void (*attachment_free)(void*) = nullptr;
};
#endif
```

### wfmash_amd/csrc/wfa_kernels.hip

```cpp
#include <hip/hip_runtime.h>
#include <stdint.h>
#include <algorithm>
#include <cstdlib>
#include <type_traits>

#include "wfa_device.h"
#include "wfa_base.h"

namespace wfm {

#ifdef WFM_PROFILE_SECTIONS
__device__ long long g_sec[8];
#define SEC_T(v) const long long v = clock64(); asm volatile("" ::: "memory")
#define SEC_ADD(i, a, b) sec[i] += (b) - (a)
#else
#define SEC_T(v)
#define SEC_ADD(i, a, b)
#endif

__device__ __forceinline__ uint64_t load8(const uint8_t* p) {
  uint64_t v;
  __builtin_memcpy(&v, p, 8);
  return v;
}
// ... 696 lines not shown
  const TileJob J = jobs[t.job];
  int touch = 0, mak = 0;
  if (x < t.n && J.s0 == t.s_k) {
    const int k = t.kmin + x;
    if (k >= -J.pl && k <= J.tl) {
      const Rng RG = make_rng(J.pl, J.tl, J.sub);
      const int64_t width = J.width;
      int32_t* rin = ring + J.ring_in + J.koff + (int64_t)t.dir * 5 * RING * width;
      const int wall = min(J.tl, J.pl + k) - t.slack;
      for (int r = 0; r < KEEP_ROWS; ++r) {
        int comp, back;
        keep_row(r, comp, back);
        const int sc = t.s_k - back;
        if (sc < 0 || k < rng_lo(RG, sc) || k > rng_hi(RG, sc)) continue;
        const int v = t.src[(int64_t)r * t.n + x];
        rin[((int64_t)(comp * RING + (sc & RMASK))) * width + k] = v;
        touch |= v >= wall;
        if (comp == C_M && v >= 0) mak = max(mak, 2 * v - k);
      }
    }
  }
  if (__any(touch) && (threadIdx.x & 63) == 0) atomicOr(&out[2 * blockIdx.y], 1);
  mak = wave_max_dpp63(mak);
  if ((threadIdx.x & 63) == 63 && mak > 0) atomicMax(&out[2 * blockIdx.y + 1], mak);
}
void launch_keep(const int32_t* ring, const TileJob* jobs, const KeepTask* tasks, int ntasks, int max_n, hipStream_t st) {
  if (ntasks <= 0 || max_n <= 0) return;
  for (int t0 = 0; t0 < ntasks; t0 += 32768)
    hipLaunchKernelGGL(wfa_keep_kernel, dim3((max_n + 255) / 256, std::min(32768, ntasks - t0)), dim3(256), 0, st, ring, jobs, tasks + t0);
}
void launch_restore(int32_t* ring, const TileJob* jobs, const RestoreTask* tasks, int32_t* out, int ntasks, int max_n, hipStream_t st) {
  if (ntasks <= 0 || max_n <= 0) return;
  for (int t0 = 0; t0 < ntasks; t0 += 32768)
    hipLaunchKernelGGL(wfa_restore_kernel, dim3((max_n + 255) / 256, std::min(32768, ntasks - t0)), dim3(256), 0, st, ring, jobs, tasks + t0, out + 2 * t0);
}

__device__ __forceinline__ const int32_t* p2_row(const int32_t* ring, const int32_t* p2, const P2Job& J, int d, int cc, int s) {
  const int sd = d == 0 ? J.sf : J.sr;
  if (s <= sd) return ring + J.ring_in + J.koff + ((int64_t)((d * 5 + cc) * RING + (s & RMASK))) * J.width;
  return p2 + J.p2_off + J.koff2 + ((int64_t)((d * 5 + cc) * P2K + (s - sd - 1))) * J.w2;
}
__device__ __forceinline__ const int32_t* p2_maxrow(const int32_t* p2max, int job, const P2Job& J, int d, int s) {
  const int sd = d == 0 ? J.sf : J.sr;
  return p2max + (((int64_t)job * 2 + d) * P2ROWS + (s - (sd - 25))) * 5;
}
__global__ __launch_bounds__(256) void wfa_p2_blockmax_kernel(const int32_t* __restrict__ ring, const int32_t* __restrict__ p2,
                                                             const P2Job* __restrict__ jobs, int32_t* __restrict__ bmax,
                                                             int32_t* __restrict__ p2max) {
  const int job = blockIdx.x / (2 * P2ROWS), r2 = blockIdx.x % (2 * P2ROWS), d = r2 / P2ROWS, r = r2 % P2ROWS;
  const P2Job J = jobs[job];
  const int s = (d == 0 ? J.sf : J.sr) - 25 + r;
  const Rng RG = make_rng(J.pl, J.tl, J.sub);
  const int lane = threadIdx.x & 63, wv = threadIdx.x >> 6, nw = blockDim.x >> 6;
  __shared__ int s_mx[5];
  if (threadIdx.x < 5) s_mx[threadIdx.x] = 0;
  __syncthreads();
  int32_t* bm = bmax + J.bm_off + ((int64_t)(d * P2ROWS + r) * 5) * J.nblk;
  int mx[5] = {0, 0, 0, 0, 0};
  const int lo = s >= 0 ? rng_lo(RG, s) : 1, hi = s >= 0 ? rng_hi(RG, s) : 0;
  const int32_t* row[5];
#pragma unroll
  for (int cc = 0; cc < 5; ++cc) row[cc] = s >= 0 ? p2_row(ring, p2, J, d, cc, s) : nullptr;
  for (int b = wv; b < J.nblk; b += nw) {
    const int k = (b << 6) - J.koff2 + lane;
    int v[5] = {0, 0, 0, 0, 0};
    if (k >= lo && k <= hi) {
#pragma unroll
      for (int cc = 0; cc < 5; ++cc) { const int o = row[cc][k]; v[cc] = o >= 0 ? 2 * o - k : 0; }
    }
#pragma unroll
    for (int cc = 0; cc < 5; ++cc) {
      const int m = wave_max_dpp63(v[cc]);
      if (lane == 63) { bm[(int64_t)cc * J.nblk + b] = m; mx[cc] = max(mx[cc], m); }
    }
  }
  if (lane == 63) {
#pragma unroll
    for (int cc = 0; cc < 5; ++cc) if (mx[cc] > 0) atomicMax(&s_mx[cc], mx[cc]);
  }
  __syncthreads();
  if (threadIdx.x < 5) p2max[(((int64_t)job * 2 + d) * P2ROWS + r) * 5 + threadIdx.x] = s_mx[threadIdx.x];
}

__global__ __launch_bounds__(256) void wfa_p2_prefixmax_kernel(const P2Job* __restrict__ jobs, const int32_t* __restrict__ bmax,
                                                              int32_t* __restrict__ pbmax, int njobs) {
  const int job = blockIdx.y;
  const P2Job J = jobs[job];
  const int e = blockIdx.x * blockDim.x + threadIdx.x;
  const int per_dir = 5 * J.nblk;
  if (e >= 2 * per_dir) return;
  const int d = e / per_dir, rest = e % per_dir;
  const int32_t* src = bmax + J.bm_off + (int64_t)d * P2ROWS * per_dir + rest;
  int32_t* dst = pbmax + J.bm_off + (int64_t)d * P2ROWS * per_dir + rest;
  int run = 0;
  for (int r = 0; r < P2ROWS; ++r) {
    run = max(run, src[(int64_t)r * per_dir]);
    dst[(int64_t)r * per_dir] = run;
  }
}

__device__ unsigned long long g_p2cnt[8];

constexpr int P2G = 8;
constexpr int P2WORK = 3072;
constexpr int P2CM = 128;
__global__ __launch_bounds__(1024) void wfa_p2_overlap_kernel(const int32_t* __restrict__ ring, const int32_t* __restrict__ p2,
                                                             const P2Job* __restrict__ jobs, const int32_t* __restrict__ p2max,
                                                             const int32_t* __restrict__ bmax, const int32_t* __restrict__ pbmax,
                                                             BpResult* __restrict__ results, DevPen pen, int scope, int count, int work_cap, int cm_max) {
  const int job = blockIdx.x, tid = threadIdx.x, lane = tid & 63, wv = tid >> 6, nw = blockDim.x >> 6;
  const P2Job J = jobs[job];
  const int nblk = J.nblk;
  const int32_t* bmj = bmax + J.bm_off;
  (void)pbmax;
  __shared__ int s_mink[P2G][P2ENT];
  __shared__ int s_k[P2G][4];
  __shared__ unsigned s_pmask[P2G][5];
  __shared__ int s_state[8];
  __shared__ int s_bp[8];
  __shared__ unsigned long long s_cells;
  __shared__ int s_rmax[2][P2ROWS][5];
  __shared__ int s_work[P2WORK][2];
  __shared__ int s_nwork, s_ovf;
  __shared__ int s_ka[P2G * 5], s_kb[P2G * 5];
  __shared__ int s_cm[P2G * 5][P2CM];
  for (int i = tid; i < 2 * P2ROWS * 5; i += blockDim.x) ((int*)s_rmax)[i] = p2max[(int64_t)job * 2 * P2ROWS * 5 + i];
  if (tid < 8) s_bp[tid] = 0;
  if (tid == 0) { s_state[0] = J.sf; s_state[1] = J.sr; s_state[2] = J.last_fwd; s_state[3] = min(J.sub < SUB_NONE ? J.sub + 1 : INT32_MAX, J.best0 > 0 ? J.best0 : INT32_MAX); s_state[4] = 0; s_state[5] = 0; s_cells = 0; }
  __syncthreads();
  const int pl = J.pl, tl = J.tl, kinv = tl - pl;
  const int aneed = tl + pl;
  const Rng RG = make_rng(pl, tl, J.sub);
  const int gopen = max(pen.o1, pen.o2);
  const long long t_begin = wall_clock64();
  long long t_cells = 0, t_list = 0, t_pick = 0;
  long long n_items = 0;
  int rounds = 0;
  for (;;) {
    ++rounds;
    const int sf0 = s_state[0], sr0 = s_state[1], lf0 = s_state[2], best = s_state[3], u0 = s_state[5];
    if (s_state[4] != 0) break;
    auto test_of = [&](int g, int& d0, int& s0, int& s1) {
      const int first = lf0 ? 0 : 1;
      const int a = first == 0 ? sf0 : sr0, b = first == 0 ? sr0 : sf0;
      if ((g & 1) == 0) { d0 = first; s0 = a + g / 2; s1 = b + g / 2; }
      else { d0 = first ^ 1; s0 = b + (g + 1) / 2; s1 = a + (g - 1) / 2; }
    };
    const int ng = min(P2G, P2TESTS - u0);
    for (int i = tid; i < P2G * P2ENT; i += blockDim.x) ((int*)s_mink)[i] = INT32_MAX;
    if (tid < P2G * 5) ((unsigned*)s_pmask)[tid] = 0u;
    if (tid < P2G) s_k[tid][2] = 0;
    __syncthreads();
    for (int e = tid; e < ng * scope * 5; e += blockDim.x) {
      const int g = e / (scope * 5), pr = e % (scope * 5), i = pr / 5, cc = pr % 5;
      int d0, s0, s1;
      test_of(g, d0, s0, s1);
      const int d1 = d0 ^ 1, sd0 = d0 == 0 ? J.sf : J.sr, sd1 = d1 == 0 ? J.sf : J.sr, si = s1 - i;
      if (si >= 0 && s0 + si - pen.o2 < best && s0 + si - bp_gap_open(pen, cc) < best &&
          s_rmax[d0][s0 - (sd0 - 25)][cc] + s_rmax[d1][si - (sd1 - 25)][cc] >= aneed) {
        atomicOr(&s_pmask[g][cc], 1u << i);
        s_k[g][2] = 1;
      }
    }
    __syncthreads();
    const long long t_c0 = wall_clock64();
    {
      if (tid == 0) { s_nwork = 0; s_ovf = 0; }
      __syncthreads();
      const long long t_l0 = wall_clock64();
      for (int it = wv; it < ng * 5; it += nw) {
        const int g = it / 5, cc = it % 5;
        const unsigned todo = s_pmask[g][cc];
        if (lane == 0) { s_ka[it] = 1; s_kb[it] = 0; }
        if (!todo) continue;
        int d0, s0, s1;
        test_of(g, d0, s0, s1);
        const int d1 = d0 ^ 1, sd0 = d0 == 0 ? J.sf : J.sr, sd1 = d1 == 0 ? J.sf : J.sr;
        int ka = INT32_MAX, kb = INT32_MIN;
        for (unsigned q = todo; q; q &= q - 1) {
          const int si = s1 - (int)__builtin_ctz(q);
          ka = min(ka, kinv - rng_hi(RG, si)); kb = max(kb, kinv - rng_lo(RG, si));
        }
        ka = max(ka, rng_lo(RG, s0)); kb = min(kb, rng_hi(RG, s0));
        if (ka > kb) continue;
        if (lane == 0) { s_ka[it] = ka; s_kb[it] = kb; }
        const int32_t* bm0 = bmj + ((int64_t)(d0 * P2ROWS + (s0 - (sd0 - 25))) * 5 + cc) * nblk;
        int M1 = 0;
        for (unsigned q = todo; q; q &= q - 1) M1 = max(M1, s_rmax[d1][s1 - (int)__builtin_ctz(q) - (sd1 - 25)][cc]);
        const bool colmax = nblk <= cm_max;
        if (colmax) {
          for (int b1 = lane; b1 < nblk; b1 += 64) {
            int cm = 0;
            for (unsigned q = todo; q; q &= q - 1) {
              const int si = s1 - (int)__builtin_ctz(q);
              cm = max(cm, bmj[((int64_t)(d1 * P2ROWS + (si - (sd1 - 25))) * 5 + cc) * nblk + b1]);
            }
            s_cm[it][b1] = cm;
// ... 134 lines not shown
        if (u >= P2TESTS) { status = 2; break; }
        const int s0 = d0 == 0 ? sf : sr, s1 = d0 == 0 ? sr : sf;
        if (count && lane == 0) { atomicAdd(&g_p2cnt[0], 1ull); if (s_k[g][2]) atomicAdd(&g_p2cnt[1], 1ull); }
        if (s_k[g][2]) {
          if (pen.o2 >= pen.o1) {
            long long key = INT64_MAX;
#pragma unroll
            for (int q = 0; q < 3; ++q) {
              const int pr = lane + 64 * q;
              if (pr < scope * 5 && s_mink[g][pr] != INT32_MAX) {
                const int i = pr / 5, cc = pr % 5, si = s1 - i;
                const int sc = s0 + si - bp_gap_open(pen, cc);
                const int oi = cc == C_D2 ? 0 : (cc == C_I2 ? 1 : (cc == C_D1 ? 2 : (cc == C_I1 ? 3 : 4)));
                if (sc < b) key = min(key, ((long long)sc << 16) | (long long)(i * 5 + oi));
              }
            }
#pragma unroll
            for (int dlt = 32; dlt >= 1; dlt >>= 1) {
              const long long o = __shfl_xor(key, dlt, 64);
              key = min(key, o);
            }
            if (key != INT64_MAX) {
              const int pos = (int)(key & 0xffff), i = pos / 5, oi = pos % 5, si = s1 - i;
              const int cc = oi == 0 ? C_D2 : (oi == 1 ? C_I2 : (oi == 2 ? C_D1 : (oi == 3 ? C_I1 : C_M)));
              const int k0 = s_mink[g][i * 5 + cc], k1 = kinv - k0;
              b = (int)(key >> 16);
              if (lane == 0) {
                s_bp[0] = b;
                if (d0 == 0) { s_bp[1] = s0; s_bp[2] = si; s_bp[3] = k0; s_bp[4] = p2_row(ring, p2, J, 0, cc, s0)[k0]; }
                else         { s_bp[1] = si; s_bp[2] = s0; s_bp[3] = k1; s_bp[4] = p2_row(ring, p2, J, 0, cc, si)[k1]; }
                s_bp[5] = cc; s_bp[7] = 1;
              }
            }
          } else {
            const int order[5] = {C_D2, C_I2, C_D1, C_I1, C_M};
            for (int i = 0; i < scope; ++i) {
              const int si = s1 - i;
              if (si < 0) break;
              for (int oi = 0; oi < 5; ++oi) {
                const int cc = order[oi];
                const int gop = bp_gap_open(pen, cc);
                if ((oi == 0 || oi == 2 || oi == 4) && s0 + si - gop >= b) break;
                const int k0 = s_mink[g][i * 5 + cc];
                if (k0 == INT32_MAX) continue;
                if (s0 + si - gop >= b) continue;
                const int k1 = kinv - k0;
                b = s0 + si - gop;
                if (lane == 0) {
                  s_bp[0] = b;
                  if (d0 == 0) { s_bp[1] = s0; s_bp[2] = si; s_bp[3] = k0; s_bp[4] = p2_row(ring, p2, J, 0, cc, s0)[k0]; }
                  else         { s_bp[1] = si; s_bp[2] = s0; s_bp[3] = k1; s_bp[4] = p2_row(ring, p2, J, 0, cc, si)[k1]; }
                  s_bp[5] = cc; s_bp[7] = 1;
                }
              }
            }
          }
        }
        if (d0 == 0) { ++sr; cells += (unsigned long long)(rng_hi(RG, sr) - rng_lo(RG, sr) + 1); last_fwd = 0; }
        else         { ++sf; cells += (unsigned long long)(rng_hi(RG, sf) - rng_lo(RG, sf) + 1); last_fwd = 1; }
        ++u;
      }
      if (lane == 0) {
        s_state[0] = sf; s_state[1] = sr; s_state[2] = last_fwd; s_state[3] = b; s_state[4] = status; s_state[5] = u;
        s_cells += cells;
      }
    }
    __syncthreads();
    t_pick += wall_clock64() - t_p0;
  }
  if (tid == 0) {
    BpResult r;
    r.status = s_state[4] == 2 ? WFM_DEV_P2_MORE : 0;
    if (r.status == 0 && !s_bp[7]) r.status = J.best0 > 0 ? WFM_DEV_P2_NOTHING : (J.sub < SUB_NONE ? WFM_DEV_BAND : WFM_DEV_UNREACHABLE);
    r.score = s_state[3]; r.score_fwd = s_bp[1]; r.score_rev = s_bp[2]; r.k_fwd = s_bp[3]; r.off_fwd = s_bp[4]; r.comp = s_bp[7] ? s_bp[5] : -1;
    r.steps = s_state[0] + s_state[1];
    r.cells = s_cells;
    r.steps_p1 = J.sf + J.sr;
    r.ticks_p1 = (uint32_t)t_cells; r.ticks_p2 = (uint32_t)(wall_clock64() - t_begin); r.pad_ = rounds;
    r.ticks_list = (uint32_t)t_list; r.ticks_pick = (uint32_t)t_pick; r.work_items = (uint32_t)n_items; r.pad2_ = 0;
    results[job] = r;
  }
}

__global__ __launch_bounds__(64) void wfa_bound_kernel(const uint8_t* __restrict__ seq, const BoundJob* __restrict__ jobs,
                                                       int32_t* __restrict__ out, DevPen pen, int njobs) {
  const int i = blockIdx.x, lane = (int)threadIdx.x;
  if (i >= njobs) return;
  const BoundJob J = jobs[i];
  const uint8_t* P = seq + J.p_off;
  const uint8_t* T = seq + J.t_off;
  const int pl = J.pl, tl = J.tl;
  auto gap = [&](int L) -> long long { return L <= 0 ? 0ll : min((long long)pen.o1 + (long long)L * pen.e1, (long long)pen.o2 + (long long)L * pen.e2); };
  auto give_up = [&]() { if (lane == 0) out[i] = -1; };
  if (min(pl, tl) < 256) { give_up(); return; }
  constexpr int PROBE = 24, RUN = 16, LOOK = 32;
  int v = 0, h = 0;
  long long score = 0;
  {
    bool found = false;
    const int amax = min(4096, max(pl, tl) - 128);
    for (int q0 = 0; q0 <= 96 && !found; q0 += 48) {
      for (int base = 0; base < amax && !found; base += 32) {
        const bool del = lane < 32;
        const int sh = base + (lane & 31);
        bool ok = false;
        if (del) {
          if (sh + q0 + PROBE <= pl && q0 + PROBE <= tl)
            ok = load8(P + sh + q0) == load8(T + q0) && load8(P + sh + q0 + 8) == load8(T + q0 + 8) && load8(P + sh + q0 + 16) == load8(T + q0 + 16);
        } else if (sh > 0) {
          if (q0 + PROBE <= pl && sh + q0 + PROBE <= tl)
            ok = load8(P + q0) == load8(T + sh + q0) && load8(P + q0 + 8) == load8(T + sh + q0 + 8) && load8(P + q0 + 16) == load8(T + sh + q0 + 16);
        }
        const unsigned long long hit = __ballot(ok);
        if (hit) {
          const unsigned hd = (unsigned)(hit & 0xffffffffull), hi = (unsigned)(hit >> 32);
          const int a = hd ? base + (int)__builtin_ctz(hd) : INT32_MAX, b = hi ? base + (int)__builtin_ctz(hi) : INT32_MAX;
          if (a <= b) { v = a; score += gap(a); } else { h = b; score += gap(b); }
          found = true;
        }
      }
    }
    if (!found) { give_up(); return; }
  }
  const int max_events = 64 + (pl + tl) / 64;
  int events = 0, forced = 0;
  for (;;) {
    const int maxn = min(pl - v, tl - h);
    int n = wave_lce_tail<false>(P, T, nullptr, nullptr, v, h, 0, maxn, lane == 0 && maxn > 0, 0, 0);
    n = rdlane(n, 0);
    v += n; h += n;
    if (v >= pl || h >= tl) break;
    if (++events > max_events) { give_up(); return; }
    int dv = 0, dh = 0;
    long long cost = 0;
    bool cand = true;
    if (lane == 0) { dv = 1; dh = 1; cost = pen.x; }
    else if (lane < 32) { dv = lane; cost = gap(lane); }
    else if (lane < 63) { dh = lane - 31; cost = gap(lane - 31); }
    else cand = false;
    const int v2 = v + dv, h2 = h + dh;
    cand = cand && v2 <= pl && h2 <= tl;
    int m = 0, mx = 0;
    if (cand) {
      mx = min(min(pl - v2, tl - h2), LOOK);
      m = min(lce_from(P + v2, T + h2, 0, mx), mx);
    }
    const bool pass = cand && (m >= RUN || m == min(pl - v2, tl - h2));
    long long key = pass ? ((cost << 8) | (long long)lane) : INT64_MAX;
#pragma unroll
    for (int d = 32; d >= 1; d >>= 1) key = min(key, __shfl_xor(key, d, 64));
    if (key != INT64_MAX) {
      const int w = (int)(key & 0xff);
      score += key >> 8;
      v += rdlane(dv, w); h += rdlane(dh, w);
      forced = 0;
    } else {
      if (++forced > 6) { give_up(); return; }
      score += pen.x; ++v; ++h;
    }
  }
  score += gap(pl - v) + gap(tl - h);
  if (lane == 0) out[i] = score < (long long)(SUB_NONE - 1) ? (int32_t)score : -1;
}
void launch_bound(const uint8_t* seq, const BoundJob* jobs, int32_t* out, int njobs, DevPen pen, hipStream_t st) {
  hipLaunchKernelGGL(wfa_bound_kernel, dim3(njobs), dim3(64), 0, st, seq, jobs, out, pen, njobs);
}
// ... 115 lines not shown
void launch_tile_init(const uint8_t* seq, int32_t* ring, const TileJob* jobs, int32_t* mak0, int njobs, int ring_rows, hipStream_t st) {
  if (ring_rows == RING) hipLaunchKernelGGL(r32::wfa_tile_init_kernel, dim3(njobs * 2), dim3(64), 0, st, seq, ring, jobs, mak0, njobs);
  else hipLaunchKernelGGL(r128::wfa_tile_init_kernel, dim3(njobs * 2), dim3(64), 0, st, seq, ring, jobs, mak0, njobs);
}
void launch_tile(const uint8_t* seq, int32_t* ring, const TileJob* jobs, const TileTask* tasks, int32_t* mak, int ntasks,
                 int threads, int T, int Wt, size_t lds_bytes, DevPen pen, int scope, int ring_rows, hipStream_t st) {
  if (ring_rows == RING) {
    (void)hipFuncSetAttribute((const void*)r32::wfa_tile_kernel, hipFuncAttributeMaxDynamicSharedMemorySize, (int)lds_bytes);
    hipLaunchKernelGGL(r32::wfa_tile_kernel, dim3(ntasks), dim3(threads), lds_bytes, st, seq, ring, jobs, tasks, mak, T, Wt, pen, scope);
  } else {
    (void)hipFuncSetAttribute((const void*)r128::wfa_tile_kernel, hipFuncAttributeMaxDynamicSharedMemorySize, (int)lds_bytes);
    hipLaunchKernelGGL(r128::wfa_tile_kernel, dim3(ntasks), dim3(threads), lds_bytes, st, seq, ring, jobs, tasks, mak, T, Wt, pen, scope);
  }
}
void launch_tile_advance(TileJob* jobs, int32_t* mak, int njobs, int T, DevPen pen, int exact, int coarse, int launched, hipStream_t st) {
  hipLaunchKernelGGL(wfa_tile_advance_kernel, dim3(njobs), dim3(64), 0, st, jobs, mak, njobs, T, pen, exact, coarse, launched);
}
void launch_tile_reg(const uint8_t* seq, int32_t* ring, const TileJob* jobs, const TileTask* tasks, int32_t* mak, int ntasks,
                     int threads, int T, int C, bool cut, hipStream_t st) {
  const size_t lds = (size_t)(T + 1) * 4;
  if (C == 4) hipLaunchKernelGGL((wfa_tile_reg_kernel<4, 256, 5, 10, 25, 2, 1>), dim3(ntasks), dim3(threads), lds, st, seq, ring, jobs, tasks, mak, T);
  else if (cut) hipLaunchKernelGGL((wfa_tile_reg_kernel<2, 1024, 5, 10, 25, 2, 1, false, true>), dim3(ntasks), dim3(threads), lds, st, seq, ring, jobs, tasks, mak, T);
  else hipLaunchKernelGGL((wfa_tile_reg_kernel<2, 1024, 5, 10, 25, 2, 1, false, false>), dim3(ntasks), dim3(threads), lds, st, seq, ring, jobs, tasks, mak, T);
}
void launch_tile_p2(const uint8_t* seq, int32_t* ring, const TileJob* jobs, const TileTask* tasks, int ntasks, int threads,
                    int32_t* p2, bool cut, hipStream_t st) {
  const size_t lds = (size_t)(P2K + 1) * 4;
  if (cut) hipLaunchKernelGGL((wfa_tile_reg_kernel<2, 1024, 5, 10, 25, 2, 1, true, true>), dim3(ntasks), dim3(threads), lds, st, seq, ring, jobs, tasks,
                              (int32_t*)nullptr, P2K, p2, (int32_t*)nullptr);
  else hipLaunchKernelGGL((wfa_tile_reg_kernel<2, 1024, 5, 10, 25, 2, 1, true, false>), dim3(ntasks), dim3(threads), lds, st, seq, ring, jobs, tasks,
                          (int32_t*)nullptr, P2K, p2, (int32_t*)nullptr);
}
__global__ __launch_bounds__(256) void wfa_p2_to_ring_kernel(int32_t* __restrict__ ring, const int32_t* __restrict__ p2, const P2Job* __restrict__ jobs) {
  const int job = blockIdx.x / (2 * 5 * RING), rest = blockIdx.x % (2 * 5 * RING), d = rest / (5 * RING), cc = (rest / RING) % 5, r = rest % RING;
  const P2Job J = jobs[job];
  const int sd = d == 0 ? J.sf : J.sr, s = sd + P2K - r;
  const Rng RG = make_rng(J.pl, J.tl, J.sub);
  const int lo = rng_lo(RG, s), hi = rng_hi(RG, s);
  const int32_t* src = p2 + J.p2_off + J.koff2 + ((int64_t)((d * 5 + cc) * P2K + (s - sd - 1))) * J.w2;
  int32_t* dst = ring + J.ring_in + ((int64_t)((d * 5 + cc) * RING + (s & RMASK))) * J.width;
  for (int c = threadIdx.x; c < J.width; c += blockDim.x) {
    const int k = c - J.koff;
    dst[c] = (k >= lo && k <= hi) ? src[k] : WF_NULL;
  }
}
void launch_p2_to_ring(int32_t* ring, const int32_t* p2, const P2Job* jobs, int njobs, hipStream_t st) {
  static_assert(P2K >= RING, "the snapshot after a round of phase 2 is taken from the P2 rows alone");
  hipLaunchKernelGGL(wfa_p2_to_ring_kernel, dim3((unsigned)njobs * 2 * 5 * RING), dim3(256), 0, st, ring, p2, jobs);
}
__global__ __launch_bounds__(256) void wfa_ring_widen_kernel(const RingWidenJob* __restrict__ jobs) {
  const RingWidenJob J = jobs[blockIdx.z];
  const int64_t c0 = ((int64_t)blockIdx.x * blockDim.x + threadIdx.x) * 4;
  if (c0 + 3 >= (int64_t)J.dst_w) return;
  const int64_t row = blockIdx.y;
  const int32_t* __restrict__ src = J.src + row * (int64_t)J.src_w;
  int32_t* __restrict__ dst = J.dst + row * (int64_t)J.dst_w;
  const int64_t delta = (int64_t)J.src_koff - J.dst_koff;
  const int64_t k0 = c0 - J.dst_koff, s0 = c0 + delta;
  int4 v = make_int4(WF_NULL, WF_NULL, WF_NULL, WF_NULL);
  const bool inside = k0 >= J.klo && k0 + 3 <= J.khi && s0 >= 0 && s0 + 3 < (int64_t)J.src_w;
  const bool aligned = ((delta & 3) == 0) && ((J.src_w & 3) == 0) && ((reinterpret_cast<uintptr_t>(J.src) & 15) == 0);
  if (inside && aligned) {
    v = *reinterpret_cast<const int4*>(src + s0);
  } else {
    int32_t e[4];
#pragma unroll
    for (int q = 0; q < 4; ++q) {
      const int64_t k = k0 + q, sc = s0 + q;
      e[q] = (k >= J.klo && k <= J.khi && sc >= 0 && sc < (int64_t)J.src_w) ? src[sc] : WF_NULL;
    }
    v = make_int4(e[0], e[1], e[2], e[3]);
  }
  if ((reinterpret_cast<uintptr_t>(J.dst) & 15) == 0) *reinterpret_cast<int4*>(dst + c0) = v;
  else { dst[c0] = v.x; dst[c0 + 1] = v.y; dst[c0 + 2] = v.z; dst[c0 + 3] = v.w; }
}
void launch_ring_widen(const RingWidenJob* jobs, int njobs, int max_dst_w, int ring_rows, hipStream_t st) {
  if (njobs <= 0 || max_dst_w <= 0) return;
  const unsigned chunks = (unsigned)((max_dst_w / 4 + 255) / 256);
  hipLaunchKernelGGL(wfa_ring_widen_kernel, dim3(chunks, (unsigned)(2 * 5 * ring_rows), (unsigned)njobs), dim3(256), 0, st, jobs);
}
void launch_p2_blockmax(const int32_t* ring, const int32_t* p2, const P2Job* jobs, int32_t* bmax, int32_t* p2max, int njobs, hipStream_t st) {
  hipLaunchKernelGGL(wfa_p2_blockmax_kernel, dim3(njobs * 2 * P2ROWS), dim3(256), 0, st, ring, p2, jobs, bmax, p2max);
}
void launch_p2_overlap(const int32_t* ring, const int32_t* p2, const P2Job* jobs, const int32_t* p2max, const int32_t* bmax, int32_t* pbmax,
                       BpResult* res, int njobs, int threads, int max_nblk, DevPen pen, int scope, hipStream_t st) {
  static const int count = getenv("WFM_P2_COUNT") ? atoi(getenv("WFM_P2_COUNT")) : 0;
  (void)max_nblk;
  static const int work_cap = getenv("WFM_P2_WORKCAP") ? std::max(1, std::min(P2WORK, atoi(getenv("WFM_P2_WORKCAP")))) : P2WORK;
  static const int cm_max = getenv("WFM_P2_COLMAX") ? std::max(0, std::min(P2CM, atoi(getenv("WFM_P2_COLMAX")))) : P2CM;
  hipLaunchKernelGGL(wfa_p2_overlap_kernel, dim3(njobs), dim3(threads), 0, st, ring, p2, jobs, p2max, bmax, pbmax, res, pen, scope, count, work_cap, cm_max);
}
void p2_counters(unsigned long long* out) { (void)hipMemcpyFromSymbol(out, HIP_SYMBOL(g_p2cnt), sizeof(unsigned long long) * 8); }
void launch_base(const uint8_t* seq, int32_t* a32, uint8_t* a8, uint32_t* rle, const BaseJob* jobs, BaseResult* res,
                 int njobs, DevPen pen, bool wide, int ring_rows, hipStream_t st) {
  if (ring_rows == RING) {
    if (wide) hipLaunchKernelGGL(r32::wfa_base_kernel<1024>, dim3(njobs), dim3(1024), 0, st, seq, a32, a8, rle, jobs, res, pen);
    else hipLaunchKernelGGL(r32::wfa_base_kernel<256>, dim3(njobs), dim3(256), 0, st, seq, a32, a8, rle, jobs, res, pen);
  } else {
    if (wide) hipLaunchKernelGGL(r128::wfa_base_kernel<1024>, dim3(njobs), dim3(1024), 0, st, seq, a32, a8, rle, jobs, res, pen);
    else hipLaunchKernelGGL(r128::wfa_base_kernel<256>, dim3(njobs), dim3(256), 0, st, seq, a32, a8, rle, jobs, res, pen);
  }
}
void launch_compact(const uint32_t* rle, const int64_t* off, const int64_t* cap, uint32_t* out, unsigned long long* total,
                    int64_t* out_start, int32_t* out_count, int nprob, hipStream_t st) {
  hipLaunchKernelGGL(rle_compact_kernel, dim3(nprob), dim3(256), 0, st, rle, off, cap, out, total, out_start, out_count);
}

}
```

### wfmash_amd/csrc/wfa_plan.h

```cpp
#ifndef WFM_WFA_PLAN_H_
#define WFM_WFA_PLAN_H_
#include <stddef.h>
#include <stdint.h>
#include <string.h>

#include <algorithm>
#include <climits>
#include <vector>

#include "../../include/wfmash_hip.h"
#include "wfa_rows.h"

namespace wfm {

struct Node {
  int32_t prob;
  int32_t pb, pl, tb, tl;
  int32_t cb, ce;
  int32_t score_rem;
  int32_t smax;
  int32_t endsfree;
  int32_t noband;
  int32_t sub;
  int32_t hinted;
// ... 201 lines not shown
    }
  }
  for (int b = 0; b < chunk; ++b) if (!p.variants_b[(size_t)b]) p.variants_b[(size_t)b] = r.planned ? 1 : 2;
}

inline int reuse_cadence(int every, int chunk) { return (std::max(1, every) + chunk - 1) / chunk * chunk; }
inline int reuse_resume_limit(int score_rem, int T, int fine_margin) {
  const int64_t x = (int64_t)score_rem / 2 - fine_margin;
  return x < 0 ? -1 : (int)(x / T * T - T);
}
inline int reuse_pick_keep(const int32_t* kept_s, size_t n, int score_rem, int T, int fine_margin, int min_blocks = 1) {
  if (score_rem == INT_MAX) return -1;
  const int limit = reuse_resume_limit(score_rem, T, fine_margin);
  const int64_t least = (int64_t)std::max(1, min_blocks) * T;
  int best = -1;
  for (size_t i = 0; i < n; ++i)
    if (kept_s[i] >= least && kept_s[i] <= limit && (best < 0 || kept_s[i] > kept_s[(size_t)best])) best = (int)i;
  return best;
}
inline bool reuse_ranges_contained(int ppl, int ptl, int psub, int cpl, int ctl, int csub, int s_k) {
  const Rng P = make_rng(ppl, ptl, psub), Cc = make_rng(cpl, ctl, csub);
  for (int s = std::max(0, s_k - RNG_BACK); s <= s_k; ++s) {
    const int lo = rng_lo(Cc, s), hi = rng_hi(Cc, s);
    if (hi < lo) continue;
    if (lo < rng_lo(P, s) || hi > rng_hi(P, s)) return false;
  }
  return true;
}
inline bool reuse_eligible(const Node& nd, const RingPlan& rp, int ppl, int ptl, int psub, int child_sub, int s_k, int T) {
  if (nd.keep <= 0 || nd.score_rem == INT_MAX || nd.sub == SUB_NONE || !rp.fits || !rp.tile_it || rp.band != 0 || rp.grown) return false;
  if (s_k < T || s_k % T != 0) return false;
  return reuse_ranges_contained(ppl, ptl, psub, nd.pl, nd.tl, child_sub, s_k);
}
inline bool reuse_keep_wanted(int es, int64_t s_meet, int cadence, int T) {
  if (s_meet <= 0) return false;
  return 100 * (int64_t)es >= 40 * s_meet - 100 * (64 + (int64_t)(2 + cadence) * T) && 100 * (int64_t)es <= 60 * s_meet;
}
inline int64_t reuse_meet_estimate(int s0, int64_t mak, int64_t A) { return s0 <= 0 || mak <= 0 ? 0 : (int64_t)s0 * A / mak; }
inline int reuse_keep_kmin(int pl, int s) { return std::max(-pl, -s); }
inline int reuse_keep_cols(int pl, int tl, int s) { return std::min(tl, s) - std::max(-pl, -s) + 1; }
inline size_t reuse_keep_elems(int pl, int tl, int s) { return (size_t)KEEP_ROWS * (size_t)reuse_keep_cols(pl, tl, s); }
struct ReuseKeeper { int pl, tl, upto; };
inline int reuse_fit_cadence(const ReuseKeeper* jobs, size_t n, int cadence, int T, size_t cap_bytes) {
  int upto_max = 0;
  for (size_t i = 0; i < n; ++i) upto_max = std::max(upto_max, jobs[i].upto);
  for (; (int64_t)cadence * T <= upto_max; cadence *= 2) {
    size_t bytes = 0;
    for (size_t i = 0; i < n && bytes <= cap_bytes; ++i)
      for (int64_t s = (int64_t)cadence * T; s <= jobs[i].upto && bytes <= cap_bytes; s += (int64_t)cadence * T) bytes += 2 * 4 * reuse_keep_elems(jobs[i].pl, jobs[i].tl, (int)s);
    if (bytes <= cap_bytes) return cadence;
  }
  return 0;
}

inline int planned_meet_sum(int score_rem, const wfm_penalties_t& pen, int comp_begin, int comp_end, bool second) {
  if (score_rem == INT_MAX || score_rem <= 0) return 0;
  const int cut = second ? comp_begin : comp_end;
  const int D = cut == 0 ? 0 : ((cut == 1 || cut == 3) ? pen.o1 : pen.o2);
  return std::max(0, score_rem - D);
}
struct PlannedMeet { int sf, sr, last_fwd; };
inline PlannedMeet planned_meet_state(int sum) { return PlannedMeet{(sum + 1) / 2, sum / 2, sum & 1}; }
inline PlannedMeet planned_meet(int score_rem, const wfm_penalties_t& pen, int comp_begin, int comp_end, bool second) {
  return planned_meet_state(planned_meet_sum(score_rem, pen, comp_begin, comp_end, second));
}
inline int planned_meet_block(int sum, int T) { return ((sum + 1) / 2 - 1) / T * T; }
inline bool planned_meet_eligible(const Node& nd, const RingPlan& rp, bool packed, int s_keep, int T) {
  if (nd.meet <= 0 || nd.score_rem == INT_MAX || nd.sub == SUB_NONE || !rp.fits || !rp.tile_it || rp.grown || !packed) return false;
  if (planned_meet_state(nd.meet).sf < 1) return false;
  return s_keep <= 0 || planned_meet_block(nd.meet, T) >= s_keep + T;
}

struct P2PlanJob { int pl, tl, sub, sf, sr, packed; };
struct P2Geometry {
  int koff2; size_t w2, nblk;
  size_t p2_off, bm_off;
};
struct P2ChunkPlan {
  std::vector<P2Geometry> geo;
  size_t elems = 0, bm_elems = 0, maxw2 = 0;
  int threads_c = 0;
  TileChunkPlan tiles;
};
inline void plan_p2_chunk(const P2PlanJob* cand, size_t n_cand, size_t i0, int rows, int rows_bm, size_t budget, int threads, int core, P2ChunkPlan& p) {
  p.geo.clear(); p.elems = 0; p.bm_elems = 0; p.maxw2 = 0;
  p.tiles.tasks.clear(); p.tiles.tasks_by.clear();
  for (size_t i = i0; i < n_cand; ++i) {
    const P2PlanJob& j = cand[i];
    const int reach = std::max(j.sf, j.sr) + rows;
    int L, R;
    rng_block(make_rng(j.pl, j.tl, j.sub), std::max(0, std::min(j.sf, j.sr) - P2_BACK), reach, L, R);
    if (R < L) { L = 0; R = 0; }
    P2Geometry g;
    g.koff2 = ((-L + 4) + 3) & ~3;
    g.w2 = ((size_t)(R + g.koff2 + 8) + 3) & ~(size_t)3;
    g.nblk = (g.w2 >> 6) + 1;
    const size_t need = g.w2 * 2 * 5 * rows, need_bm = g.nblk * 2 * rows_bm * 5;
    if (!p.geo.empty() && (p.elems + need + 2 * (p.bm_elems + need_bm)) * 4 > budget) break;
    p.maxw2 = std::max(p.maxw2, g.w2);
    g.p2_off = p.elems; g.bm_off = p.bm_elems;
    p.bm_elems += need_bm;
    p.elems += need;
    p.geo.push_back(g);
  }
  const size_t n = p.geo.size();
  auto dir_range = [&](const P2PlanJob& j, int d, int& L, int& R) { rng_block(make_rng(j.pl, j.tl, j.sub), d == 0 ? j.sf : j.sr, (d == 0 ? j.sf : j.sr) + rows, L, R); };
  p.threads_c = threads; p.tiles.core_c = core;
  int widest = 0;
  for (size_t q = 0; q < n; ++q)
    for (int d = 0; d < 2; ++d) {
      int L, R;
      dir_range(cand[i0 + q], d, L, R);
      widest = std::max(widest, R - L + 1);
    }
  if (fits_one_tile(widest, threads, 2)) {
    p.threads_c = one_tile_threads(widest, threads, 2);
    p.tiles.core_c = p.threads_c * 2;
  }
  for (size_t q = 0; q < n; ++q)
    for (int d = 0; d < 2; ++d) {
      int L, R;
      dir_range(cand[i0 + q], d, L, R);
      append_tile_tasks(p.tiles, (int)q, d, tiles_for(L, R, p.tiles.core_c), p.tiles.core_c, cand[i0 + q].packed != 0);
    }
  close_task_list(p.tiles);
}

inline void base_columns(const Node& nd, int pbf, int pef, int tbf, int tef, bool corner_band, int64_t* kmin_out, int64_t* kmax_out) {
  int64_t kmin = nd.endsfree ? std::max<int64_t>(-nd.pl, -(int64_t)pbf - nd.smax) : std::max<int64_t>(-nd.pl, -nd.smax);
  int64_t kmax = nd.endsfree ? std::min<int64_t>(nd.tl, (int64_t)tbf + nd.smax) : std::min<int64_t>(nd.tl, nd.smax);
  const bool end_fixed = !nd.endsfree || (pef == 0 && tef == 0);
  if (corner_band && end_fixed) {
    const int64_t k_end = (int64_t)nd.tl - nd.pl;
    const int64_t bmin = std::max(kmin, k_end - nd.smax), bmax = std::min(kmax, k_end + nd.smax);
    const int64_t lo0 = nd.endsfree ? std::max<int64_t>(-(int64_t)pbf, bmin) : 0, hi0 = nd.endsfree ? std::min<int64_t>((int64_t)tbf, bmax) : 0;
    if (bmin <= bmax && lo0 <= hi0 && lo0 >= bmin && hi0 <= bmax) { kmin = bmin; kmax = bmax; }
  }
  *kmin_out = kmin; *kmax_out = kmax;
}

struct BaseRules {
  bool base_v2 = true;
  bool base_tiles = true;
  bool force_tiles = false;
  bool few_jobs = false;
  int wide_from = 2048;
};
inline int base_kind(int64_t width, int pl, int tl, int tries, bool acgt, const BaseRules& r) {
  if (r.base_v2 && (pl == 0 || tl == 0)) return 1;
  if (r.base_v2 && width <= 2048 && acgt)
    return width <= 128 ? 0 : (r.base_tiles && (r.force_tiles || (r.few_jobs && (tries > 0 || width > 640))) ? 5 : (width <= 640 ? 1 : 2));
  if (r.base_v2 && r.base_tiles && acgt) return 5;
  return width > r.wide_from ? 4 : 3;
}

struct BaseTilePlan { int core = 0, nblocks = 0; std::vector<int> ntiles; };
inline BaseTilePlan plan_base_tiles(const int32_t* width, const int32_t* smax, size_t n, int T, int threads) {
  BaseTilePlan p;
  p.core = threads * 2 - 2 * T;
  p.ntiles.resize(n);
  int smax_all = 0;
  for (size_t q = 0; q < n; ++q) {
    p.ntiles[q] = (width[q] + p.core - 1) / p.core;
    smax_all = std::max(smax_all, smax[q]);
  }
  p.nblocks = (smax_all + T - 1) / T + 1;
  return p;
}

enum { EXPAND_OK = 0, EXPAND_SPANS = 1, EXPAND_ARENA = 2, EXPAND_RUN_TOO_LONG = 3 };
struct Expanded {
  int32_t score = -1;
  uint32_t n_runs = 0, ops_len = 0;
  uint64_t pc = 0, tc = 0;
};
inline int expand_runs(const uint32_t* e, int cnt, const wfm_penalties_t& pen, int plen, int tlen, char* ops, size_t ops_cap,
                       std::vector<uint32_t>* runs_out, Expanded* out) {
  static const char opc[4] = {'M', 'X', 'I', 'D'};
  const size_t runs_before = runs_out ? runs_out->size() : 0;
  int64_t score = 0;
  uint64_t pc = 0, tc = 0, both = 0;
  uint32_t nruns = 0;
  size_t pos = 0;
  int k = 0;
  while (k < cnt) {
    const int op = (int)(e[k] & 3u);
    uint64_t len = e[k] >> 2;
    int k2 = k + 1;
    while (k2 < cnt && (int)(e[k2] & 3u) == op) { len += e[k2] >> 2; ++k2; }
    if (runs_out) {
      if (len >= (1u << 30)) return EXPAND_RUN_TOO_LONG;
      runs_out->push_back((uint32_t)(len << 2) | (uint32_t)op);
    } else {
      if (pos + len > ops_cap) return EXPAND_ARENA;
      memset(ops + pos, opc[op], (size_t)len);
      pos += (size_t)len;
    }
    ++nruns;
    if (op == 1) { score += (int64_t)len * pen.x; pc += len; tc += len; both += len; }
    else if (op == 0) { pc += len; tc += len; both += len; }
    else {
      score += std::min<int64_t>(pen.o1 + (int64_t)len * pen.e1, pen.o2 + (int64_t)len * pen.e2);
      if (op == 2) tc += len; else pc += len;
    }
    k = k2;
  }
  out->pc = pc; out->tc = tc;
  if (pc != (uint64_t)plen || tc != (uint64_t)tlen) {
// ... 12 lines not shown
```

Measured before the change: 64.57 million aligned bases/s.

## Add exact-score phase-2 walk that skips block-max search for planned meets

When the planner already knows the final score (resume_s + resume_sr equals the planned meet, best0 is zero, penalties ordered), phase-2 jobs are routed to a new kernel. That kernel tests only the overlap rows implied by the known score, instead of running the blockmax and overlap search. Jobs are reordered so search jobs come first and exact jobs after, and the block-maxima buffers are sized only for search jobs. Exact misses fall back to a second search launch, which costs an extra host sync round trip; the unused pbmax buffer is also removed.

```diff
diff --git a/include/wfmash_hip.h b/include/wfmash_hip.h
--- a/include/wfmash_hip.h
+++ b/include/wfmash_hip.h
@@ -270,7 +270,9 @@
   WFM_TC_REUSE_TOUCHED = 11,
   WFM_TC_REUSE_FELL_OTHER = 12,
   WFM_TC_PLANNED_ENDS = 13,
-  WFM_TILE_COUNTERS = 14
+  WFM_TC_P2_EXACT = 14,
+  WFM_TC_P2_EXACT_MISSES = 15,
+  WFM_TILE_COUNTERS = 16
 };
 size_t wfm_get_tile_counters(const wfm_handle_t* h, uint64_t* out, size_t n);
 
diff --git a/wfmash_amd/capi.py b/wfmash_amd/capi.py
--- a/wfmash_amd/capi.py
+++ b/wfmash_amd/capi.py
@@ -18,7 +18,8 @@
 WFM_PF_ROOT_AGAIN, WFM_PF_JOB_AGAIN, WFM_PF_BASE_RETRY, WFM_PF_BASE_RETRY2, WFM_PF_BYTE_KERNEL, WFM_PF_P2_ROUNDS, WFM_PF_RING_KERNEL, WFM_PF_BASE_TILES = 1, 2, 4, 8, 16, 32, 64, 128
 WFM_PF_RING_GROWN = 256
 TILE_COUNTERS = ("jobs", "exact_ends", "fine_reruns", "gap_reruns", "ring3", "blocks_coarse", "blocks_fine", "left_band",
-                 "reuse_resumed", "reuse_fallbacks", "reuse_keeps", "reuse_touched", "reuse_fell_other", "planned_ends")
+                 "reuse_resumed", "reuse_fallbacks", "reuse_keeps", "reuse_touched", "reuse_fell_other", "planned_ends",
+                 "p2_exact", "p2_exact_misses")
 
 EXPORTS = [
     "wfm_create", "wfm_destroy", "wfm_last_error", "wfm_device_name",
diff --git a/wfmash_amd/csrc/wfa_device.h b/wfmash_amd/csrc/wfa_device.h
--- a/wfmash_amd/csrc/wfa_device.h
+++ b/wfmash_amd/csrc/wfa_device.h
@@ -23,6 +23,7 @@
 constexpr int WFM_DEV_P2_NOTHING = -6;
 constexpr int WFM_DEV_LIMIT = -7;
 constexpr int WFM_DEV_P2_MORE = -5;
+constexpr int WFM_DEV_P2_EXACT_MISS = -8;
 
 struct DevPen { int x, o1, e1, o2, e2; };
 
@@ -113,8 +114,10 @@
   int32_t sf, sr, last_fwd;
   int32_t sub, best0;
   int32_t nblk;
+  int32_t exact;
   int64_t bm_off;
 };
+static_assert(sizeof(P2Job) == 80, "P2Job is built by the host per launch: nothing else holds its layout");
 
 struct BpResult {
   int32_t status;
@@ -299,8 +302,9 @@
 };
 void launch_ring_widen(const RingWidenJob* jobs, int njobs, int max_dst_w, int ring_rows, hipStream_t st);
 void launch_p2_blockmax(const int32_t* ring, const int32_t* p2, const P2Job* jobs, int32_t* bmax, int32_t* p2max, int njobs, hipStream_t st);
-void launch_p2_overlap(const int32_t* ring, const int32_t* p2, const P2Job* jobs, const int32_t* p2max, const int32_t* bmax, int32_t* pbmax,
+void launch_p2_overlap(const int32_t* ring, const int32_t* p2, const P2Job* jobs, const int32_t* p2max, const int32_t* bmax,
                        BpResult* res, int njobs, int threads, int max_nblk, DevPen pen, int scope, hipStream_t st);
+void launch_p2_exact(const int32_t* ring, const int32_t* p2, const P2Job* jobs, BpResult* res, int njobs, int threads, DevPen pen, int scope, hipStream_t st);
 void launch_base(const uint8_t* seq, int32_t* a32, uint8_t* a8, uint32_t* rle, const BaseJob* jobs, BaseResult* res,
                  int njobs, DevPen pen, bool wide, int ring_rows, hipStream_t st);
 void launch_compact(const uint32_t* rle, const int64_t* off, const int64_t* cap, uint32_t* out, unsigned long long* total,
diff --git a/wfmash_amd/csrc/wfa_host.hip b/wfmash_amd/csrc/wfa_host.hip
--- a/wfmash_amd/csrc/wfa_host.hip
+++ b/wfmash_amd/csrc/wfa_host.hip
@@ -880,20 +880,28 @@
   wfm_handle* h; wfm_seqset* S; const DevPen& dp; int scope; const TileCfg& cfg; std::vector<BpJob>& jobs;
   const std::vector<int>& cand; const std::vector<int64_t>& ring_other; std::vector<BpResult>& res; double& ms_out;
   std::vector<BpResult>& carry; std::vector<char>& has_carry; bool may_continue; std::vector<int>& again;
+  const std::vector<int32_t>& exact_of;
   std::vector<P2PlanJob> pcand;
+  std::vector<char> pexact;
   P2ChunkPlan plan;
   size_t i0 = 0, n = 0;
   std::vector<TileJob> tj;
   std::vector<P2Job> pj;
+  std::vector<int> at;
+  std::vector<P2Job> pj_dev;
+  size_t ns = 0, ns_dump = 0;
   std::vector<BpResult> got;
   float ms = 0;
 };
 
 void fill_p2_chunk(P2Chunk& c, size_t i0) {
   const size_t budget = std::max<size_t>(c.h->mem_budget / 4, (size_t)64 << 20);
-  plan_p2_chunk(c.pcand.data(), c.pcand.size(), i0, P2K, P2ROWS, budget, c.cfg.threads, c.cfg.Wt - 2 * P2K, c.plan);
+  plan_p2_chunk(c.pcand.data(), c.pcand.size(), i0, P2K, P2ROWS, budget, c.cfg.threads, c.cfg.Wt - 2 * P2K, c.plan, c.pexact.data());
   c.i0 = i0; c.n = c.plan.geo.size();
   c.tj.clear(); c.pj.clear();
+  c.at.assign(c.n, 0); c.ns = 0;
+  for (size_t q = 0; q < c.n; ++q) c.ns += !c.pexact[i0 + q];
+  for (size_t q = 0, s = 0, e = c.ns; q < c.n; ++q) c.at[q] = (int)(c.pexact[i0 + q] ? e++ : s++);
   for (size_t q = 0; q < c.n; ++q) {
     const BpJob& j = c.jobs[(size_t)c.cand[i0 + q]];
     const P2Geometry& g = c.plan.geo[q];
@@ -904,54 +912,98 @@
     P2Job pq{};
     pq.ring_in = j.ring_off; pq.p2_off = (int64_t)g.p2_off; pq.width = j.width; pq.koff = j.koff; pq.w2 = (int32_t)g.w2; pq.koff2 = g.koff2;
     pq.pl = j.pl; pq.tl = j.tl; pq.sf = j.resume_s; pq.sr = j.resume_sr; pq.last_fwd = j.last_fwd; pq.sub = j.sub; pq.best0 = j.best0;
-    pq.nblk = (int32_t)g.nblk; pq.bm_off = (int64_t)g.bm_off;
+    pq.nblk = (int32_t)g.nblk; pq.bm_off = (int64_t)g.bm_off; pq.exact = c.exact_of[i0 + q];
     c.tj.push_back(t); c.pj.push_back(pq);
   }
+  c.pj_dev.resize(c.n);
+  for (size_t q = 0; q < c.n; ++q) c.pj_dev[(size_t)c.at[q]] = c.pj[q];
 }
 
 int launch_p2_chunk(P2Chunk& c) {
   wfm_handle* h = c.h;
   wfm_seqset* S = c.S;
-  const size_t n = c.n, elems = c.plan.elems, bm_elems = c.plan.bm_elems, n_pk = c.plan.tiles.n_pk;
+  const size_t n = c.n, ns = c.ns, elems = c.plan.elems, bm_elems = c.plan.bm_elems, n_pk = c.plan.tiles.n_pk;
   const std::vector<TileTask>& tasks = c.plan.tiles.tasks;
   const int threads_c = c.plan.threads_c;
-  if (h->p2rows.ensure(elems + 16) || h->p2max.ensure(n * 2 * P2ROWS * 5) || h->p2bmax.ensure(bm_elems + 16) || h->p2pbmax.ensure(bm_elems + 16) ||
+  if (h->p2rows.ensure(elems + 16) || h->p2max.ensure(ns * 2 * P2ROWS * 5) || h->p2bmax.ensure(bm_elems + 16) ||
       h->p2jobs.ensure(n) || h->tilejobs.ensure(n) || h->tiletasks.ensure(tasks.size()) || h->bpres.ensure(std::max(n, c.jobs.size()))) {
     h->err = "out of device memory (phase-2 rows)"; return WFM_E_NOMEM;
   }
   HIPCHK(h, hipMemcpyAsync(h->tilejobs.p, c.tj.data(), n * sizeof(TileJob), hipMemcpyHostToDevice, h->stream));
-  HIPCHK(h, hipMemcpyAsync(h->p2jobs.p, c.pj.data(), n * sizeof(P2Job), hipMemcpyHostToDevice, h->stream));
+  HIPCHK(h, hipMemcpyAsync(h->p2jobs.p, c.pj_dev.data(), n * sizeof(P2Job), hipMemcpyHostToDevice, h->stream));
   HIPCHK(h, hipMemcpyAsync(h->tiletasks.p, tasks.data(), tasks.size() * sizeof(TileTask), hipMemcpyHostToDevice, h->stream));
   HIPCHK(h, hipEventRecord(h->ev0, h->stream));
   bool any_cut = false;
   for (const TileJob& t : c.tj) any_cut |= t.sub != SUB_NONE;
   if (n_pk) launch_tile2_p2(S->d_pk, h->ring.p, h->tilejobs.p, h->tiletasks.p, (int)n_pk, threads_c, h->p2rows.p, h->stream);
   if (tasks.size() > n_pk) launch_tile_p2(S->d_seq, h->ring.p, h->tilejobs.p, h->tiletasks.p + n_pk, (int)(tasks.size() - n_pk), threads_c, h->p2rows.p, any_cut, h->stream);
-  launch_p2_blockmax(h->ring.p, h->p2rows.p, h->p2jobs.p, h->p2bmax.p, h->p2max.p, (int)n, h->stream);
   static const int p2_threads = getenv("WFM_P2_THREADS") ? atoi(getenv("WFM_P2_THREADS")) : 0;
-  launch_p2_overlap(h->ring.p, h->p2rows.p, h->p2jobs.p, h->p2max.p, h->p2bmax.p, h->p2pbmax.p, h->bpres.p, (int)n,
-                    p2_threads > 0 ? p2_threads : 1024, (int)(c.plan.maxw2 >> 6) + 1, c.dp, c.scope, h->stream);
+  static const int p2x_threads = getenv("WFM_P2_EXACT_THREADS") ? atoi(getenv("WFM_P2_EXACT_THREADS")) : 0;
+  auto launch_search = [&](size_t cnt) {
+    launch_p2_blockmax(h->ring.p, h->p2rows.p, h->p2jobs.p, h->p2bmax.p, h->p2max.p, (int)cnt, h->stream);
+    launch_p2_overlap(h->ring.p, h->p2rows.p, h->p2jobs.p, h->p2max.p, h->p2bmax.p, h->bpres.p, (int)cnt,
+                      p2_threads > 0 ? p2_threads : 1024, (int)(c.plan.maxw2 >> 6) + 1, c.dp, c.scope, h->stream);
+  };
+  if (ns) launch_search(ns);
+  launch_p2_exact(h->ring.p, h->p2rows.p, h->p2jobs.p + ns, h->bpres.p + ns, (int)(n - ns), p2x_threads > 0 ? p2x_threads : p2_exact_threads(c.plan.maxw2), c.dp, c.scope, h->stream);
   HIPCHK(h, hipGetLastError());
   HIPCHK(h, hipEventRecord(h->ev1, h->stream));
-  c.got.resize(n);
-  HIPCHK(h, hipMemcpyAsync(c.got.data(), h->bpres.p, n * sizeof(BpResult), hipMemcpyDeviceToHost, h->stream));
+  std::vector<BpResult> dev(n);
+  HIPCHK(h, hipMemcpyAsync(dev.data(), h->bpres.p, n * sizeof(BpResult), hipMemcpyDeviceToHost, h->stream));
   HIPCHK(h, hipStreamSynchronize(h->stream));
   HIPCHK(h, hipEventElapsedTime(&c.ms, h->ev0, h->ev1));
+  auto note_busy = [&](float ms) {
+    if (!h->call_base) return hipSuccess;
+    float t0 = 0;
+    const hipError_t e = hipEventElapsedTime(&t0, h->call_base, h->ev0);
+    if (e == hipSuccess) h->bp_iv.emplace_back(t0, t0 + ms);
+    return e;
+  };
+  HIPCHK(h, note_busy(c.ms));
+  c.got.resize(n);
+  for (size_t q = 0; q < n; ++q) c.got[q] = dev[(size_t)c.at[q]];
+  c.ns_dump = ns;
+  h->tile_ctr[WFM_TC_P2_EXACT] += n - ns;
+  std::vector<size_t> miss;
+  for (size_t q = 0; q < n; ++q) if (c.got[q].status == WFM_DEV_P2_EXACT_MISS) miss.push_back(q);
+  if (!miss.empty()) {
+    h->tile_ctr[WFM_TC_P2_EXACT_MISSES] += miss.size();
+    std::vector<P2Job> mj;
+    size_t bm = 0;
+    for (size_t q : miss) {
+      P2Job& pq = c.pj[q];
+      pq.exact = 0; pq.bm_off = (int64_t)bm;
+      bm += (size_t)pq.nblk * 2 * P2ROWS * 5;
+      mj.push_back(pq);
+    }
+    if (h->p2max.ensure(mj.size() * 2 * P2ROWS * 5) || h->p2bmax.ensure(bm + 16)) { h->err = "out of device memory (phase-2 maxima)"; return WFM_E_NOMEM; }
+    HIPCHK(h, hipMemcpyAsync(h->p2jobs.p, mj.data(), mj.size() * sizeof(P2Job), hipMemcpyHostToDevice, h->stream));
+    HIPCHK(h, hipEventRecord(h->ev0, h->stream));
+    launch_search(mj.size());
+    HIPCHK(h, hipGetLastError());
+    HIPCHK(h, hipEventRecord(h->ev1, h->stream));
+    HIPCHK(h, hipMemcpyAsync(dev.data(), h->bpres.p, mj.size() * sizeof(BpResult), hipMemcpyDeviceToHost, h->stream));
+    HIPCHK(h, hipStreamSynchronize(h->stream));
+    float ms2 = 0;
+    HIPCHK(h, hipEventElapsedTime(&ms2, h->ev0, h->ev1));
+    HIPCHK(h, note_busy(ms2));
+    c.ms += ms2;
+    for (size_t m = 0; m < miss.size(); ++m) c.got[miss[m]] = dev[m];
+    c.ns_dump = 0;
+  }
   c.ms_out += c.ms;
-  if (h->call_base) {
-    float t0 = 0;
-    HIPCHK(h, hipEventElapsedTime(&t0, h->call_base, h->ev0));
-    h->bp_iv.emplace_back(t0, t0 + c.ms);
-  }
   return WFM_OK;
 }
 
 int dump_p2_job(P2Chunk& c) {
   wfm_handle* h = c.h;
   const std::vector<BpResult>& got = c.got;
-  const size_t q = std::min<size_t>((size_t)c.cfg.p2_dump, c.n - 1);
+  if (c.ns_dump == 0) { fprintf(stderr, "[wfm] p2 dump: no job of this chunk of %zu searches with its row maxima at hand (%zu take the exact walk)\n", c.n, c.n - c.ns); return WFM_OK; }
+  const size_t pos = std::min<size_t>((size_t)c.cfg.p2_dump, c.ns_dump - 1);
+  size_t q = 0;
+  while ((size_t)c.at[q] != pos) ++q;
   std::vector<int32_t> rm((size_t)2 * P2ROWS * 5);
-  HIPCHK(h, hipMemcpy(rm.data(), h->p2max.p + q * 2 * P2ROWS * 5, rm.size() * 4, hipMemcpyDeviceToHost));
+  HIPCHK(h, hipMemcpy(rm.data(), h->p2max.p + pos * 2 * P2ROWS * 5, rm.size() * 4, hipMemcpyDeviceToHost));
   const P2Job& pjq = c.pj[q];
   fprintf(stderr, "[wfm] p2 dump job %zu: pl %d tl %d sf %d sr %d last_fwd %d sub %d w2 %d nblk %d -> status %d score %d (fwd %d rev %d comp %d k %d) rounds %d\n", q, pjq.pl, pjq.tl, pjq.sf,
           pjq.sr, pjq.last_fwd, pjq.sub, pjq.w2, pjq.nblk, got[q].status, got[q].score, got[q].score_fwd, got[q].score_rev, got[q].comp, got[q].k_fwd, got[q].pad_);
@@ -970,8 +1022,14 @@
   int more = 0;
   double tk = 0, tc = 0, rd = 0; uint32_t tkmax = 0; int rdmax = 0;
   for (const BpResult& r : got) { more += r.status == WFM_DEV_P2_MORE; tk += r.ticks_p2; tc += r.ticks_p1; rd += r.pad_; tkmax = std::max(tkmax, r.ticks_p2); rdmax = std::max(rdmax, r.pad_); }
-  fprintf(stderr, "[wfm] phase 2 from rows computed ahead: %zu jobs, widest %zu columns, %zu tiles of %d threads, %.3f ms, %d left to the step kernel; walk per job: %.1f rounds (max %d), %.0f us (max %.0f), of which cells stage %.0f us\n",
-          n, c.plan.maxw2, c.plan.tiles.tasks.size(), c.plan.threads_c, c.ms, more, rd / n, rdmax, tk / n / 100.0, tkmax / 100.0, tc / n / 100.0);
+  double tests = 0; int tests_max = 0;
+  for (const BpResult& r : got) { tests += r.steps - r.steps_p1; tests_max = std::max(tests_max, r.steps - r.steps_p1); }
+  size_t missed = 0;
+  for (size_t q = 0; q < n; ++q) missed += pj[q].exact == 0 && (size_t)c.at[q] >= c.ns;
+  fprintf(stderr, "[wfm] phase 2 from rows computed ahead: %zu jobs, widest %zu columns, %zu tiles of %d threads, %.3f ms, %d left to the step kernel; walk per job: %.1f rounds (max %d), %.0f us (max %.0f), of which cells stage %.0f us; "
+          "%.1f tests (max %d); exact walk %.1f %% of the jobs, missed %.1f %%\n",
+          n, c.plan.maxw2, c.plan.tiles.tasks.size(), c.plan.threads_c, c.ms, more, rd / n, rdmax, tk / n / 100.0, tkmax / 100.0, tc / n / 100.0, tests / n, tests_max,
+          100.0 * (n - c.ns) / n, 100.0 * missed / n);
   size_t qs = 0;
   for (size_t q = 0; q < n; ++q) if (got[q].ticks_p2 > got[qs].ticks_p2) qs = q;
   fprintf(stderr, "[wfm]   slowest walk: pl %d tl %d sub %d w2 %d nblk %d: %d rounds, %.0f us = listing %.0f + cells %.0f (incl. listing) + pick %.0f, %u blocks listed, status %d\n", pj[qs].pl, pj[qs].tl,
@@ -1009,12 +1067,13 @@
 
 int run_p2_phase(wfm_handle* h, wfm_seqset* S, const DevPen& dp, int scope, const TileCfg& cfg, std::vector<BpJob>& jobs,
                  const std::vector<int>& cand, const std::vector<int64_t>& ring_other, std::vector<BpResult>& res, double& ms_out,
-                 std::vector<BpResult>& carry, std::vector<char>& has_carry, bool may_continue, std::vector<int>& again) {
+                 std::vector<BpResult>& carry, std::vector<char>& has_carry, bool may_continue, std::vector<int>& again, const std::vector<int32_t>& exact_of) {
   if (cand.empty()) return WFM_OK;
-  P2Chunk c{h, S, dp, scope, cfg, jobs, cand, ring_other, res, ms_out, carry, has_carry, may_continue, again};
-  for (int q : cand) {
-    const BpJob& j = jobs[(size_t)q];
+  P2Chunk c{h, S, dp, scope, cfg, jobs, cand, ring_other, res, ms_out, carry, has_carry, may_continue, again, exact_of};
+  for (size_t i = 0; i < cand.size(); ++i) {
+    const BpJob& j = jobs[(size_t)cand[i]];
     c.pcand.push_back(P2PlanJob{j.pl, j.tl, j.sub, j.resume_s, j.resume_sr, j.packed});
+    c.pexact.push_back((char)(exact_of[i] > 0));
   }
   for (size_t i0 = 0; i0 < cand.size(); i0 += c.n) {
     fill_p2_chunk(c, i0);
@@ -1036,6 +1095,7 @@
   bool use_bound = use_hints && num("WFM_BOUND", 1) != 0;
   int slack_env = num("WFM_SUB_SLACK", -1);
   bool ring3_on = num("WFM_TILE_RING3", 1) != 0, p2_on = num("WFM_P2", 1) != 0;
+  bool p2_exact = num("WFM_P2_EXACT", 1) != 0;
   int p2_rounds = std::max(1, num("WFM_P2_ROUNDS", 64));
   int fine_margin = num("WFM_TILE_FINE_MARGIN", 48);
   int coarse_min_blocks = num("WFM_TILE_COARSE_MIN_BLOCKS", 32), coarse_max_jobs = num("WFM_TILE_COARSE_MAX_JOBS", 128);
@@ -1377,11 +1437,17 @@
   k.rest.clear(); k.more_set.clear();
   std::vector<int> cand;
   std::vector<int64_t> other;
+  std::vector<int32_t> exact_of;
   std::vector<char> is_cand(k.jobs.size(), 0);
   if (c.knobs.p2_on && c.tcfg.reg && c.tcfg.exact)
     for (size_t q = 0; q < k.tiled.size(); ++q) {
       const BpJob& j = k.jobs[(size_t)k.tiled[q]];
-      if (j.resume_s >= 0 && j.resume_sr >= 0) { cand.push_back(k.tiled[q]); other.push_back(k.ring2[q]); is_cand[(size_t)k.tiled[q]] = 1; }
+      if (j.resume_s >= 0 && j.resume_sr >= 0) {
+        cand.push_back(k.tiled[q]); other.push_back(k.ring2[q]); is_cand[(size_t)k.tiled[q]] = 1;
+        const bool exact = c.knobs.p2_exact && q < k.plan_from.size() && k.plan_from[q] > 0 && j.resume_s + j.resume_sr == k.plan_from[q] && j.best0 == 0 &&
+                           c.dp.o2 >= c.dp.o1 && c.dp.o1 >= 0;
+        exact_of.push_back(exact ? k.plan_from[q] : 0);
+      }
     }
   double pms = 0;
   k.carry.assign(k.jobs.size(), BpResult{});
@@ -1390,7 +1456,8 @@
   std::vector<int64_t> other_r = other;
   for (int round = 1; !cand_r.empty(); ++round) {
     again.clear();
-    const int rc = run_p2_phase(h, c.S, c.dp, c.scope, c.tcfg, k.jobs, cand_r, other_r, k.res, pms, k.carry, k.has_carry, round < c.knobs.p2_rounds, again);
+    if (round > 1) exact_of.assign(cand_r.size(), 0);
+    const int rc = run_p2_phase(h, c.S, c.dp, c.scope, c.tcfg, k.jobs, cand_r, other_r, k.res, pms, k.carry, k.has_carry, round < c.knobs.p2_rounds, again, exact_of);
     if (rc != WFM_OK) return rc;
     std::vector<int> c2; std::vector<int64_t> o2;
     for (int a : again) {
@@ -1839,7 +1906,7 @@
   if (h->stage) { (void)hipHostFree(h->stage); h->stage = nullptr; h->stage_cap = 0; }
   for (int k = 0; k < 2; ++k)
     if (h->cspin[k]) { (void)hipHostFree(h->cspin[k]); h->cspin[k] = nullptr; }
-  h->p2rows.release(); h->p2max.release(); h->p2bmax.release(); h->p2pbmax.release(); h->p2jobs.release(); h->widenjobs.release(); h->keeptasks.release(); h->restoretasks.release(); h->restoreres.release();
+  h->p2rows.release(); h->p2max.release(); h->p2bmax.release(); h->p2jobs.release(); h->widenjobs.release(); h->keeptasks.release(); h->restoretasks.release(); h->restoreres.release();
   h->bpjobs.release(); h->bpres.release(); h->bsjobs.release(); h->bsres.release();
   h->b2tjobs.release(); h->b2ttasks.release(); h->b2tkeys.release(); h->b2toffs.release(); h->b2tactive.release();
   h->i64a.release(); h->i64b.release(); h->i64c.release(); h->i32a.release(); h->seqflags.release(); h->flagjobs.release(); h->gathertasks.release(); h->scratch.release(); h->outblk.release(); h->optrows.release(); h->total.release();
diff --git a/wfmash_amd/csrc/wfa_host_shared.h b/wfmash_amd/csrc/wfa_host_shared.h
--- a/wfmash_amd/csrc/wfa_host_shared.h
+++ b/wfmash_amd/csrc/wfa_host_shared.h
@@ -112,7 +112,7 @@
   wfm::DevBuf<wfm::TileJob> tilejobs;
   wfm::DevBuf<wfm::TileTask> tiletasks;
   wfm::DevBuf<int32_t> tilemak;
-  wfm::DevBuf<int32_t> p2rows, p2max, p2bmax, p2pbmax;
+  wfm::DevBuf<int32_t> p2rows, p2max, p2bmax;
   wfm::DevBuf<wfm::P2Job> p2jobs;
   wfm::DevBuf<wfm::RingWidenJob> widenjobs;
   wfm::DevBuf<wfm::KeepTask> keeptasks;
diff --git a/wfmash_amd/csrc/wfa_kernels.hip b/wfmash_amd/csrc/wfa_kernels.hip
--- a/wfmash_amd/csrc/wfa_kernels.hip
+++ b/wfmash_amd/csrc/wfa_kernels.hip
@@ -802,23 +802,6 @@
   if (threadIdx.x < 5) p2max[(((int64_t)job * 2 + d) * P2ROWS + r) * 5 + threadIdx.x] = s_mx[threadIdx.x];
 }
 
-__global__ __launch_bounds__(256) void wfa_p2_prefixmax_kernel(const P2Job* __restrict__ jobs, const int32_t* __restrict__ bmax,
-                                                              int32_t* __restrict__ pbmax, int njobs) {
-  const int job = blockIdx.y;
-  const P2Job J = jobs[job];
-  const int e = blockIdx.x * blockDim.x + threadIdx.x;
-  const int per_dir = 5 * J.nblk;
-  if (e >= 2 * per_dir) return;
-  const int d = e / per_dir, rest = e % per_dir;
-  const int32_t* src = bmax + J.bm_off + (int64_t)d * P2ROWS * per_dir + rest;
-  int32_t* dst = pbmax + J.bm_off + (int64_t)d * P2ROWS * per_dir + rest;
-  int run = 0;
-  for (int r = 0; r < P2ROWS; ++r) {
-    run = max(run, src[(int64_t)r * per_dir]);
-    dst[(int64_t)r * per_dir] = run;
-  }
-}
-
 __device__ unsigned long long g_p2cnt[8];
 
 constexpr int P2G = 8;
@@ -826,13 +809,12 @@
 constexpr int P2CM = 128;
 __global__ __launch_bounds__(1024) void wfa_p2_overlap_kernel(const int32_t* __restrict__ ring, const int32_t* __restrict__ p2,
                                                              const P2Job* __restrict__ jobs, const int32_t* __restrict__ p2max,
-                                                             const int32_t* __restrict__ bmax, const int32_t* __restrict__ pbmax,
+                                                             const int32_t* __restrict__ bmax,
                                                              BpResult* __restrict__ results, DevPen pen, int scope, int count, int work_cap, int cm_max) {
   const int job = blockIdx.x, tid = threadIdx.x, lane = tid & 63, wv = tid >> 6, nw = blockDim.x >> 6;
   const P2Job J = jobs[job];
   const int nblk = J.nblk;
   const int32_t* bmj = bmax + J.bm_off;
-  (void)pbmax;
   __shared__ int s_mink[P2G][P2ENT];
   __shared__ int s_k[P2G][4];
   __shared__ unsigned s_pmask[P2G][5];
@@ -1133,6 +1115,116 @@
   }
 }
 
+__global__ __launch_bounds__(1024) void wfa_p2_exact_kernel(const int32_t* __restrict__ ring, const int32_t* __restrict__ p2, const P2Job* __restrict__ jobs,
+                                                           BpResult* __restrict__ results, DevPen pen, int scope, int reach) {
+  const int job = blockIdx.x, tid = threadIdx.x;
+  const P2Job J = jobs[job];
+  __shared__ int s_mink[P2G * 5];
+  __shared__ int s_end[2];
+  __shared__ int s_bp[8];
+  __shared__ unsigned long long s_cells;
+  if (tid == 0) { s_end[0] = 0; s_end[1] = 0; s_cells = 0; }
+  if (tid < 8) s_bp[tid] = 0;
+  __syncthreads();
+  const int pl = J.pl, tl = J.tl, kinv = tl - pl;
+  const Rng RG = make_rng(pl, tl, J.sub);
+  const int n_tests = min(min(scope + max(pen.o1, pen.o2), P2TESTS), reach);
+  auto test_of = [&](int u, int& d0, int& s0, int& s1) {
+    const int first = J.last_fwd ? 0 : 1;
+    const int a = first == 0 ? J.sf : J.sr, b = first == 0 ? J.sr : J.sf;
+    if ((u & 1) == 0) { d0 = first; s0 = a + u / 2; s1 = b + u / 2; }
+    else { d0 = first ^ 1; s0 = b + (u + 1) / 2; s1 = a + (u - 1) / 2; }
+  };
+  auto row_of = [&](int s0, int s1, int cc) {
+    const int i = s0 + s1 - bp_gap_open(pen, cc) - J.exact;
+    return (i >= 0 && i < scope && s1 - i >= 0) ? i : -1;
+  };
+  const long long t_begin = wall_clock64();
+  long long t_cells = 0, t_pick = 0;
+  int rounds = 0;
+  for (;;) {
+    const int u0 = s_end[1];
+    if (s_end[0] != 0) break;
+    ++rounds;
+    const int ng = min(P2G, n_tests - u0);
+    if (tid < P2G * 5) s_mink[tid] = INT32_MAX;
+    __syncthreads();
+    const long long t_c0 = wall_clock64();
+    for (int it = 0; it < ng * 5; ++it) {
+      const int g = it / 5, cc = it % 5;
+      int d0, s0, s1;
+      test_of(u0 + g, d0, s0, s1);
+      const int i = row_of(s0, s1, cc);
+      if (i < 0) continue;
+      const int si = s1 - i;
+      const int ka = max(rng_lo(RG, s0), kinv - rng_hi(RG, si)), kb = min(rng_hi(RG, s0), kinv - rng_lo(RG, si));
+      if (ka > kb) continue;
+      const int32_t* R0 = p2_row(ring, p2, J, d0, cc, s0);
+      const int32_t* R1 = p2_row(ring, p2, J, d0 ^ 1, cc, si) + kinv;
+      int mk = INT32_MAX;
+      for (int kk = ka + tid; kk <= kb; kk += 4 * (int)blockDim.x) {
+        int o0[4], o1[4];
+#pragma unroll
+        for (int j = 0; j < 4; ++j) {
+          const int k0 = kk + j * (int)blockDim.x;
+          o0[j] = k0 <= kb ? R0[k0] : WF_NULL;
+          o1[j] = k0 <= kb ? R1[-k0] : WF_NULL;
+        }
+#pragma unroll
+        for (int j = 3; j >= 0; --j)
+          if (o0[j] + o1[j] >= tl) mk = min(mk, kk + j * (int)blockDim.x);
+      }
+      if (mk != INT32_MAX) atomicMin(&s_mink[it], mk);
+    }
+    __syncthreads();
+    t_cells += wall_clock64() - t_c0;
+    const long long t_p0 = wall_clock64();
+    if (tid == 0) {
+      unsigned long long cells = 0;
+      int status = 0, u = u0;
+      for (int g = 0; g < ng; ++g, ++u) {
+        int d0, s0, s1;
+        test_of(u, d0, s0, s1);
+        int key = INT32_MAX;
+        for (int cc = 0; cc < 5; ++cc) {
+          if (s_mink[g * 5 + cc] == INT32_MAX) continue;
+          const int oi = cc == C_D2 ? 0 : (cc == C_I2 ? 1 : (cc == C_D1 ? 2 : (cc == C_I1 ? 3 : 4)));
+          key = min(key, row_of(s0, s1, cc) * 5 + oi);
+        }
+        if (key != INT32_MAX) {
+          const int i = key / 5, oi = key % 5, si = s1 - i;
+          const int cc = oi == 0 ? C_D2 : (oi == 1 ? C_I2 : (oi == 2 ? C_D1 : (oi == 3 ? C_I1 : C_M)));
+          const int k0 = s_mink[g * 5 + cc], k1 = kinv - k0;
+          if (d0 == 0) { s_bp[1] = s0; s_bp[2] = si; s_bp[3] = k0; s_bp[4] = p2_row(ring, p2, J, 0, cc, s0)[k0]; }
+          else         { s_bp[1] = si; s_bp[2] = s0; s_bp[3] = k1; s_bp[4] = p2_row(ring, p2, J, 0, cc, si)[k1]; }
+          s_bp[5] = cc;
+          status = 1;
+          break;
+        }
+        const int sn = s1 + 1;
+        cells += (unsigned long long)(rng_hi(RG, sn) - rng_lo(RG, sn) + 1);
+      }
+      if (status == 0 && u >= n_tests) status = 2;
+      s_end[0] = status; s_end[1] = u;
+      s_cells += cells;
+    }
+    __syncthreads();
+    t_pick += wall_clock64() - t_p0;
+  }
+  if (tid == 0) {
+    BpResult r;
+    const bool hit = s_end[0] == 1;
+    r.status = hit ? 0 : WFM_DEV_P2_EXACT_MISS;
+    r.score = J.exact; r.score_fwd = s_bp[1]; r.score_rev = s_bp[2]; r.k_fwd = s_bp[3]; r.off_fwd = s_bp[4]; r.comp = hit ? s_bp[5] : -1;
+    r.steps = J.sf + J.sr + s_end[1];
+    r.cells = s_cells;
+    r.steps_p1 = J.sf + J.sr;
+    r.ticks_p1 = (uint32_t)t_cells; r.ticks_p2 = (uint32_t)(wall_clock64() - t_begin); r.pad_ = rounds;
+    r.ticks_list = 0; r.ticks_pick = (uint32_t)t_pick; r.work_items = 0; r.pad2_ = 0;
+    results[job] = r;
+  }
+}
+
 __global__ __launch_bounds__(64) void wfa_bound_kernel(const uint8_t* __restrict__ seq, const BoundJob* __restrict__ jobs,
                                                        int32_t* __restrict__ out, DevPen pen, int njobs) {
   const int i = blockIdx.x, lane = (int)threadIdx.x;
@@ -1414,13 +1506,19 @@
 void launch_p2_blockmax(const int32_t* ring, const int32_t* p2, const P2Job* jobs, int32_t* bmax, int32_t* p2max, int njobs, hipStream_t st) {
   hipLaunchKernelGGL(wfa_p2_blockmax_kernel, dim3(njobs * 2 * P2ROWS), dim3(256), 0, st, ring, p2, jobs, bmax, p2max);
 }
-void launch_p2_overlap(const int32_t* ring, const int32_t* p2, const P2Job* jobs, const int32_t* p2max, const int32_t* bmax, int32_t* pbmax,
+void launch_p2_overlap(const int32_t* ring, const int32_t* p2, const P2Job* jobs, const int32_t* p2max, const int32_t* bmax,
                        BpResult* res, int njobs, int threads, int max_nblk, DevPen pen, int scope, hipStream_t st) {
   static const int count = getenv("WFM_P2_COUNT") ? atoi(getenv("WFM_P2_COUNT")) : 0;
   (void)max_nblk;
   static const int work_cap = getenv("WFM_P2_WORKCAP") ? std::max(1, std::min(P2WORK, atoi(getenv("WFM_P2_WORKCAP")))) : P2WORK;
   static const int cm_max = getenv("WFM_P2_COLMAX") ? std::max(0, std::min(P2CM, atoi(getenv("WFM_P2_COLMAX")))) : P2CM;
-  hipLaunchKernelGGL(wfa_p2_overlap_kernel, dim3(njobs), dim3(threads), 0, st, ring, p2, jobs, p2max, bmax, pbmax, res, pen, scope, count, work_cap, cm_max);
+  hipLaunchKernelGGL(wfa_p2_overlap_kernel, dim3(njobs), dim3(threads), 0, st, ring, p2, jobs, p2max, bmax, res, pen, scope, count, work_cap, cm_max);
+}
+void launch_p2_exact(const int32_t* ring, const int32_t* p2, const P2Job* jobs, BpResult* res, int njobs, int threads, DevPen pen, int scope, hipStream_t st) {
+  if (njobs <= 0) return;
+  const char* e = getenv("WFM_P2_EXACT_REACH");
+  const int reach = e ? std::max(1, atoi(e)) : P2TESTS;
+  hipLaunchKernelGGL(wfa_p2_exact_kernel, dim3(njobs), dim3(std::max(64, std::min(1024, threads & ~63))), 0, st, ring, p2, jobs, res, pen, scope, reach);
 }
 void p2_counters(unsigned long long* out) { (void)hipMemcpyFromSymbol(out, HIP_SYMBOL(g_p2cnt), sizeof(unsigned long long) * 8); }
 void launch_base(const uint8_t* seq, int32_t* a32, uint8_t* a8, uint32_t* rle, const BaseJob* jobs, BaseResult* res,
diff --git a/wfmash_amd/csrc/wfa_plan.h b/wfmash_amd/csrc/wfa_plan.h
--- a/wfmash_amd/csrc/wfa_plan.h
+++ b/wfmash_amd/csrc/wfa_plan.h
@@ -307,7 +307,8 @@
   int threads_c = 0;
   TileChunkPlan tiles;
 };
-inline void plan_p2_chunk(const P2PlanJob* cand, size_t n_cand, size_t i0, int rows, int rows_bm, size_t budget, int threads, int core, P2ChunkPlan& p) {
+inline void plan_p2_chunk(const P2PlanJob* cand, size_t n_cand, size_t i0, int rows, int rows_bm, size_t budget, int threads, int core, P2ChunkPlan& p,
+                          const char* exact = nullptr) {
   p.geo.clear(); p.elems = 0; p.bm_elems = 0; p.maxw2 = 0;
   p.tiles.tasks.clear(); p.tiles.tasks_by.clear();
   for (size_t i = i0; i < n_cand; ++i) {
@@ -320,7 +321,7 @@
     g.koff2 = ((-L + 4) + 3) & ~3;
     g.w2 = ((size_t)(R + g.koff2 + 8) + 3) & ~(size_t)3;
     g.nblk = (g.w2 >> 6) + 1;
-    const size_t need = g.w2 * 2 * 5 * rows, need_bm = g.nblk * 2 * rows_bm * 5;
+    const size_t need = g.w2 * 2 * 5 * rows, need_bm = (exact && exact[i]) ? 0 : g.nblk * 2 * rows_bm * 5;
     if (!p.geo.empty() && (p.elems + need + 2 * (p.bm_elems + need_bm)) * 4 > budget) break;
     p.maxw2 = std::max(p.maxw2, g.w2);
     g.p2_off = p.elems; g.bm_off = p.bm_elems;
@@ -349,6 +350,11 @@
       append_tile_tasks(p.tiles, (int)q, d, tiles_for(L, R, p.tiles.core_c), p.tiles.core_c, cand[i0 + q].packed != 0);
     }
   close_task_list(p.tiles);
+}
+
+inline int p2_exact_threads(size_t maxw2) {
+  const size_t t = ((maxw2 + 3) / 4 + 63) / 64 * 64;
+  return (int)std::min<size_t>(1024, std::max<size_t>(128, t));
 }
 
 inline void base_columns(const Node& nd, int pbf, int pef, int tbf, int tef, bool corner_band, int64_t* kmin_out, int64_t* kmax_out) {
```

Result: faster. 69.41 million aligned bases/s (median of 6 runs) (+7.5%).
